# slowkoni/InStruct

Measured on AMD Instinct MI355X. Metric: MCMC iterations/sec (update_P+update_ZQ+update_SG) at NxLxK, higher is better.
Workload: dtype f64; 1 GPU; config3: N=10000 L=5000 K=5 diploid mode 2, 1 chain per GPU; N=10000, L=5000, K=5, ploidy=2, mode=2, rng_schedule=replay, chains=1, parallelism=1 independent chain(s), one per GPU

## Files before the change

### instruct_amd/csrc/isg_hip.hip

```cpp
#include <hip/hip_runtime.h>
#include <limits.h>
#include <math.h>
#include <stdint.h>
#include <stdio.h>
#include <stdlib.h>
#include <string.h>
#include <atomic>
#include <chrono>
#include <string>
#include <thread>
#include <vector>
#include <new>
#include <type_traits>
#include "../../include/instruct_hip.h"
#include "isg_math.h"
#include "isg_wh.h"
#include "isg_sampler.h"
#include "isg_host_dirichlet.h"
#include "isg_kdispatch.h"
#include "isg_devbuf.h"

#define ISG_KCAP 32
#define ISG_KWIDE 64
#define ISG_LPT 4

static thread_local std::string g_err;
static int fail(const std::string &m)
{
	g_err = m;
	return 1;
}
static bool env_flag(const char *e, bool def) { return e ? (def ? atoi(e) != 0 : atoi(e) == 1) : def; }
static long env_int(const char *e, long def, long lo = LONG_MIN, long hi = LONG_MAX) { return (e && atol(e) >= lo && atol(e) <= hi) ? atol(e) : def; }
static double env_double(const char *e, double def, double lo, double hi = HUGE_VAL) { return (e && atof(e) >= lo && atof(e) <= hi) ? atof(e) : def; }
#define HIPCHK(x)                                                                                     \
	do {                                                                                          \
		hipError_t e_ = (x);                                                                  \
		if (e_ != hipSuccess)                                                                 \
			return fail(std::string(#x) + ": " + hipGetErrorString(e_));                  \
	} while (0)

struct DevView {
	int N, L, Lp, K, KP, Amax, mode, type_freq;
	const uint8_t *geno;
	uint8_t *z;
	const int *allelenum;
	const int *nvalid;
	const unsigned *rankwave;
	int nwv;
	double *freq;
	float *freqf;
	int KPF;
	double *lftab, *lltab;
	int2 *lli;
	unsigned lli_F;
	const double *tape;
	unsigned long long tape_len;
	int *cnt;
	double *qq;
	int *qqnum;
	int *gen;
	int *genprop;
	double *uacc;
	double *indvlkh;
	const isg_wh_tables *tab;
	unsigned *err;
};

struct ProfEntry {
	std::string name;
	double ms;
	long n;
};
struct ProfPending {
	const char *name;
	hipEvent_t e0, e1;
};

struct PolyCtx;
struct InbreedCtx;
struct ResolveCtx;
struct PDevCtx;
struct SpecCtx;
template <class T>
struct PageAlloc {
	typedef T value_type;
	PageAlloc() {}
	template <class U> PageAlloc(const PageAlloc<U> &) {}
	T *allocate(size_t n)
	{
		void *p = nullptr;
		const size_t bytes = (n * sizeof(T) + 4095) & ~(size_t)4095;
		if (posix_memalign(&p, 4096, bytes ? bytes : 4096)) throw std::bad_alloc();
		return (T *)p;
	}
	void deallocate(T *p, size_t) { free(p); }
	template <class U> bool operator==(const PageAlloc<U> &) const { return true; }
	template <class U> bool operator!=(const PageAlloc<U> &) const { return false; }
};
template <class T> using hvec = std::vector<T, PageAlloc<T>>;

struct CoopBuf;
struct CtxBufs {
	DevBuf<uint8_t> d_geno, d_z;
	DevBuf<int> d_allelenum, d_nvalid, d_cnt, d_qqnum, d_gen, d_genprop;
	DevBuf<unsigned> d_rankwave;
	DevBuf<double> d_freq, d_lftab, d_lltab, d_qq, d_uacc, d_indvlkh;
	DevBuf<float> d_freqf;
	DevBuf<int2> d_lli;
	DevBuf<isg_wh_tables> d_tab;
	DevBuf<uint64_t> d_pos;
	DevBuf<unsigned> d_err;
	DevBuf<double> d_S;
	DevBuf<double> d_Fprop;
	DevBuf<double> d_tape;
	DevBuf<CoopBuf> d_coop;
	DevBuf<unsigned long long> d_pipe;
	DevBuf<unsigned long long> d_spop;
	DevBuf<double> d_qqsave;
	DevBuf<int> d_state;
	DevBuf<double> d_ratios, d_total;
	PinnedBuf<double> htape;
	DevEvent ev_tape;
	DevEvent ev_cnt;
	DevBuf<double> st_qq, st_qq2, st_lkh, st_gen, st_gen2, st_freq, st_freq2;
};
struct isg_ctx : CtxBufs {
	isg_config cfg;
	ResolveCtx *rs = nullptr;
	SpecCtx *zspec = nullptr;
	PDevCtx *pdev = nullptr;
	PolyCtx *poly = nullptr;
	InbreedCtx *inb = nullptr;
	DevView d;
	int Amax;
	hipStream_t stream;
	std::vector<int> allelenum;
	hvec<double> freq;
	hvec<double> qq;
	hvec<int> qqnum;
	hvec<int> gen;
	hvec<double> S;
	hvec<int> state;
	hvec<double> indvlkh;
	hvec<int> cnt_h;
	hvec<double> freq_stage;
	double alpha, totallkh;
	isg_wh rng;
	isg_wh origin;
	long raw_seed[3];
	bool raw_valid;
	uint64_t iter;
	uint64_t ky[9];
	isg_wh_tables tab_h;
	uint64_t nvalid_total;
	int coop;
	int spec;
	int xcd;
	int pipe;
	int pipe_xcd;
	bool counted = false;
	double host_t[8] = {0, 0, 0, 0, 0, 0, 0, 0};
	long host_n = 0;
	bool host_timing = false;
	std::vector<void *> pinned;
	bool ahead_valid = false;
	isg_wh ahead_rng;
	std::vector<double> pshape;
	std::vector<HostGammaCoef> pcoef;
	uint64_t htape_len = 0;
	int host_tape = 1;
	int spop_tree = 1;
	int test_abort = 0;
	long zq_fallbacks = 0;
	hvec<double> ratios_h;
	bool h_qq, h_gen, h_S, h_lkh;
	long st_step = 0;
	bool st_on = false;
	bool prof;
	std::vector<ProfEntry> prof_entries;
	std::vector<ProfPending> prof_pending;
	std::vector<hipEvent_t> prof_free;
	hipEvent_t prof_cur;
};


__device__ __forceinline__ unsigned lane_id() { return threadIdx.x & 63u; }

__device__ __forceinline__ unsigned wave_sum_u32(unsigned x)
{
	x += (unsigned)__builtin_amdgcn_update_dpp(0, (int)x, 0x121, 0xf, 0xf, false);
	x += (unsigned)__builtin_amdgcn_update_dpp(0, (int)x, 0x122, 0xf, 0xf, false);
	x += (unsigned)__builtin_amdgcn_update_dpp(0, (int)x, 0x124, 0xf, 0xf, false);
	x += (unsigned)__builtin_amdgcn_update_dpp(0, (int)x, 0x128, 0xf, 0xf, false);
	return (unsigned)__builtin_amdgcn_readlane((int)x, 0) + (unsigned)__builtin_amdgcn_readlane((int)x, 16) +
	       (unsigned)__builtin_amdgcn_readlane((int)x, 32) + (unsigned)__builtin_amdgcn_readlane((int)x, 48);
}


template <int BLOCK>
__device__ __forceinline__ unsigned block_excl_scan(unsigned v, unsigned *sm , unsigned *total)
{
	const int NW = BLOCK / 64;
	unsigned lane = lane_id(), w = threadIdx.x >> 6, incl = v;
#pragma unroll
	for (int o = 1; o < 64; o <<= 1) {
		unsigned t = __shfl_up(incl, o, 64);
		if (lane >= (unsigned)o) incl += t;
	}
	if (lane == 63) sm[w] = incl;
	__syncthreads();
	unsigned base = 0, tot = 0;
#pragma unroll
	for (int i = 0; i < NW; i++) {
		unsigned s = sm[i];
		if (i < (int)w) base += s;
		tot += s;
	}
	__syncthreads();
	*total = tot;
	return base + incl - v;
}

struct AccLimbs {
	unsigned long long l0, l1, l2, l3;
	unsigned flags;
};
__device__ __forceinline__ AccLimbs acc_to_limbs(const isg_acc &a)
{
	AccLimbs r;
	r.l0 = a.lo & 0xffffffffULL;
	r.l1 = a.lo >> 32;
	r.l2 = a.hi & 0xffffffffULL;
	r.l3 = a.hi >> 32;
	r.flags = a.flags;
	return r;
}
__device__ __forceinline__ isg_acc limbs_to_acc(const AccLimbs &s)
{
	isg_acc a;
	unsigned long long t0 = s.l0, t1 = s.l1 + (t0 >> 32), t2 = s.l2 + (t1 >> 32), t3 = s.l3 + (t2 >> 32);
	a.lo = (t0 & 0xffffffffULL) | (t1 << 32);
	a.hi = (t2 & 0xffffffffULL) | (t3 << 32);
	a.flags = s.flags;
	return a;
}
template <int BLOCK>
__device__ __forceinline__ isg_acc block_reduce_acc(const isg_acc &a, unsigned long long *sm )
{
	const int NW = BLOCK / 64;
	AccLimbs s = acc_to_limbs(a);
#pragma unroll
	for (int o = 32; o > 0; o >>= 1) {
		s.l0 += __shfl_down(s.l0, o, 64);
		s.l1 += __shfl_down(s.l1, o, 64);
		s.l2 += __shfl_down(s.l2, o, 64);
		s.l3 += __shfl_down(s.l3, o, 64);
		s.flags |= __shfl_down(s.flags, o, 64);
	}
	unsigned w = threadIdx.x >> 6;
	if (lane_id() == 0) {
		sm[w * 5 + 0] = s.l0;
		sm[w * 5 + 1] = s.l1;
		sm[w * 5 + 2] = s.l2;
		sm[w * 5 + 3] = s.l3;
		sm[w * 5 + 4] = s.flags;
	}
	__syncthreads();
	AccLimbs t = {0, 0, 0, 0, 0};
	for (int i = 0; i < NW; i++) {
		t.l0 += sm[i * 5 + 0];
		t.l1 += sm[i * 5 + 1];
		t.l2 += sm[i * 5 + 2];
		t.l3 += sm[i * 5 + 3];
		t.flags |= (unsigned)sm[i * 5 + 4];
	}
	__syncthreads();
	return limbs_to_acc(t);
}

template <int BLOCK, int LPT>
__global__ void __launch_bounds__(BLOCK) k_count(DevView d, int rows_per_block)
{
	extern __shared__ unsigned lds_cnt[];
	const int C = LPT * d.Amax * d.K;
	const int t = threadIdx.x;
	for (int c = 0; c < C; c++) lds_cnt[c * BLOCK + t] = 0;
	const int J0 = blockIdx.x * BLOCK * LPT;
	const int j0 = J0 + t * LPT;
	const int r0 = blockIdx.y * rows_per_block;
	int r1 = r0 + rows_per_block;
	if (r1 > d.N) r1 = d.N;
	const size_t rowb = (size_t)d.Lp * 2;
	if (j0 < d.Lp) {
		for (int i = r0; i < r1; i++) {
			unsigned long long gb, zb;
			if (LPT == 4) {
				const uint2 g = *(const uint2 *)(d.geno + (size_t)i * rowb + (size_t)j0 * 2);
				const uint2 zz = *(const uint2 *)(d.z + (size_t)i * rowb + (size_t)j0 * 2);
				gb = ((unsigned long long)g.y << 32) | g.x;
				zb = ((unsigned long long)zz.y << 32) | zz.x;
			} else {
				gb = *(const unsigned short *)(d.geno + (size_t)i * rowb + (size_t)j0 * 2);
				zb = *(const unsigned short *)(d.z + (size_t)i * rowb + (size_t)j0 * 2);
			}
#pragma unroll
			for (int l = 0; l < LPT; l++) {
				unsigned a0 = (unsigned)(gb >> (16 * l)) & 0xff, a1 = (unsigned)(gb >> (16 * l + 8)) & 0xff;
				unsigned z0 = (unsigned)(zb >> (16 * l)) & 0xff, z1 = (unsigned)(zb >> (16 * l + 8)) & 0xff;
				if (a0 != 0xff) {
					lds_cnt[((l * d.Amax + a0) * d.K + z0) * BLOCK + t] += 1;
					lds_cnt[((l * d.Amax + a1) * d.K + z1) * BLOCK + t] += 1;
				}
			}
		}
	}
	__syncthreads();
	const int per_locus = d.Amax * d.K;
	int tile_loci = d.L - J0;
	if (tile_loci > BLOCK * LPT) tile_loci = BLOCK * LPT;
	if (tile_loci < 0) tile_loci = 0;
	const int E = tile_loci * per_locus;
	for (int e = t; e < E; e += BLOCK) {
		int jl = e / per_locus, rem = e - jl * per_locus;
		unsigned v = lds_cnt[((jl % LPT) * per_locus + rem) * BLOCK + jl / LPT];
		if (v) atomicAdd(&d.cnt[(size_t)J0 * per_locus + e], (int)v);
	}
}

__global__ void k_count_atomic(DevView d)
{
	const size_t id = (size_t)blockIdx.x * blockDim.x + threadIdx.x;
	if (id >= (size_t)d.N * d.Lp) return;
	const unsigned short g = ((const unsigned short *)d.geno)[id], z = ((const unsigned short *)d.z)[id];
	const unsigned a0 = g & 0xff, a1 = g >> 8;
	if (a0 == 0xff) return;
	const size_t j = id % d.Lp;
	atomicAdd(&d.cnt[(j * d.Amax + a0) * d.K + (z & 0xff)], 1);
	atomicAdd(&d.cnt[(j * d.Amax + a1) * d.K + (z >> 8)], 1);
}

template <int BLOCK, int KC>
__device__ __forceinline__ void gprop_body(DevView d, const double *S, isg_wh base, int keyed, uint64_t *pos_out)
{
	__shared__ unsigned sm[BLOCK / 64 + 1];
	__shared__ double Ssh[KC];
	const bool indiv = (d.mode == 3);
	if (!indiv && threadIdx.x < (unsigned)d.K) Ssh[threadIdx.x] = S[threadIdx.x];
	__syncthreads();
	unsigned running = 0;
	for (int i0 = 0; i0 < d.N; i0 += BLOCK) {
		int i = i0 + threadIdx.x;
		double selfing = 0;
		int stat = 0;
		if (i < d.N) {
			if (indiv) selfing = S[i];
			else for (int k = 0; k < d.K; k++) selfing += d.qq[(size_t)i * d.K + k] * Ssh[k];
			stat = isg_dt_stat(selfing);
			if (stat < 0) {
				if ((atomicOr(d.err, 2u) & 2u) == 0u) *(double *)(d.err + 2) = selfing;
				stat = 1;
			}
		}
		unsigned flag = (i < d.N && stat == 1) ? 1u : 0u, tot, pre;
		pre = block_excl_scan<BLOCK>(flag, sm, &tot);
		if (i < d.N) {
			uint64_t pos = keyed ? 2ull * (uint64_t)i : (uint64_t)i + running + pre;
			isg_cursor c;
			c.s = isg_wh_jump(d.tab, base, pos);
			c.used = 0;
			c.tape = nullptr;
			int gen;
			if (stat == 1) {
				gen = isg_rgeom(&c, 1 - selfing);
				if (gen < 1) gen = 1;
				if (gen > 50) gen = 50;
			} else if (stat == 0) gen = 1;
			else gen = 50;
			d.genprop[i] = gen;
			d.uacc[i] = isg_cur_next(&c);
		}
		running += tot;
	}
	if (threadIdx.x == 0) *pos_out = (uint64_t)d.N + running;
}
template <int BLOCK>
__global__ void __launch_bounds__(BLOCK) k_gprop(DevView d, const double *S, isg_wh base, int keyed, uint64_t *pos_out) { gprop_body<BLOCK, ISG_KCAP>(d, S, base, keyed, pos_out); }
template <int BLOCK>
__global__ void __launch_bounds__(BLOCK) k_gprop_w(DevView d, const double *S, isg_wh base, int keyed, uint64_t *pos_out) { gprop_body<BLOCK, ISG_KWIDE>(d, S, base, keyed, pos_out); }

template <int BLOCK>
__device__ __forceinline__ isg_acc2 block_reduce_acc2(const isg_acc2 &a, long long *sm )
{
	const int NW = BLOCK / 64;
	long long hi = a.hi, lo = a.lo;
	unsigned fl = a.flags;
#pragma unroll
	for (int o = 32; o > 0; o >>= 1) {
		hi += __shfl_down(hi, o, 64);
		lo += __shfl_down(lo, o, 64);
		fl |= __shfl_down(fl, o, 64);
	}
	const unsigned w = threadIdx.x >> 6;
	if (lane_id() == 0) {
		sm[w * 3 + 0] = hi;
		sm[w * 3 + 1] = lo;
		sm[w * 3 + 2] = (long long)fl;
	}
	__syncthreads();
	isg_acc2 r;
	r.hi = 0;
	r.lo = 0;
	r.flags = 0;
	for (int i = 0; i < NW; i++) {
		r.hi += sm[i * 3 + 0];
		r.lo += sm[i * 3 + 1];
		r.flags |= (unsigned)sm[i * 3 + 2];
	}
	__syncthreads();
	return r;
}

__global__ void k_lltab(DevView d)
{
	const size_t id = (size_t)blockIdx.x * blockDim.x + threadIdx.x;
	const size_t per = (size_t)d.L * d.Amax * d.Amax * d.K;
	if (id >= per) return;
	const int k = (int)(id % d.K);
	const int a1 = (int)((id / d.K) % d.Amax), a0 = (int)((id / d.K / d.Amax) % d.Amax), j = (int)(id / d.K / d.Amax / d.Amax);
	const double f0 = d.freq[((size_t)j * d.Amax + a0) * d.KP + k], f1 = d.freq[((size_t)j * d.Amax + a1) * d.KP + k];
	if (a1 == 0) d.lftab[((size_t)j * d.Amax + a0) * d.K + k] = isg_log(f0);
	if (!d.lltab || d.mode != 2) return;
	if (a0 == a1) {
		double result = f0 * f0, temp = 2 * f0 * (1 - f0);
		for (int g = 1; g <= 50; g++) {
			d.lltab[(size_t)(g - 1) * per + id] = isg_log(result);
			temp /= 2;
			result += temp / 2;
		}
	} else {
		for (int g = 1; g <= 50; g++) d.lltab[(size_t)(g - 1) * per + id] = isg_log(2 * f0 * f1 * isg_scalbn(1.0, -(g - 1)));
	}
}

__device__ __forceinline__ int2 lli_entry(double v)
{
	if (!(v > -1024.0 && v < 1024.0)) {
		const uint64_t u = isg_d2u(v);
		return make_int2((int)0x80000000u, (u == 0x7ff0000000000000ULL) ? 1 : (u == 0xfff0000000000000ULL) ? 2 : 4);
	}
	const double hs = __builtin_rint(v * 1048576.0);
	const double lo = isg_fma(hs, -0x1p-20, v);
	return make_int2((int)hs, (int)__builtin_rint(lo * 0x1p51));
}
__global__ void k_lltab_int(DevView d)
{
	const size_t id = (size_t)blockIdx.x * blockDim.x + threadIdx.x;
	const size_t AAK = (size_t)d.Amax * d.Amax * d.K;
	if (id == 0) d.lli[0] = make_int2(0, 0);
	if (id >= AAK * d.L) return;
	const int j = (int)(id % d.L), combo = (int)(id / d.L);
	const int k = combo % d.K, a1 = (combo / d.K) % d.Amax, a0 = combo / d.K / d.Amax;
	const double f0 = d.freq[((size_t)j * d.Amax + a0) * d.KP + k], f1 = d.freq[((size_t)j * d.Amax + a1) * d.KP + k];
	if (a1 == 0) d.lli[d.lli_F + ((size_t)a0 * d.K + k) * d.Lp + j] = lli_entry(isg_log(f0));
	int2 *out = d.lli + 1 + (size_t)combo * d.Lp + j;
	const size_t gstride = AAK * d.Lp;
	if (a0 == a1) {
		double result = f0 * f0, temp = 2 * f0 * (1 - f0);
		for (int g = 1; g <= 50; g++) {
			out[(size_t)(g - 1) * gstride] = lli_entry(isg_log(result));
			temp /= 2;
			result += temp / 2;
		}
	} else {
		for (int g = 1; g <= 50; g++) out[(size_t)(g - 1) * gstride] = lli_entry(isg_log(2 * f0 * f1 * isg_scalbn(1.0, -(g - 1))));
	}
}

// ... 960 lines not shown
	if (a == 2) return (b == 2 || b == 1) ? 0.5 : 0.0;
	if (a == 1) return (b == 0 || b == 2) ? 0.05 : (b == 1 ? 0.90 : 0.0);
	return 0.0;
}
template <int BLOCK>
__device__ __forceinline__ double dev_proposal(const DevView &d, const double *s, unsigned long long *smr)
{
	isg_acc a;
	isg_acc_zero(&a);
	for (int i = threadIdx.x; i < d.N; i += BLOCK) {
		double temp = 0;
		for (int j = 0; j < d.K; j++) temp += d.qq[(size_t)i * d.K + j] * s[j];
		isg_acc_add(&a, isg_log(isg_pow(temp, (double)(d.gen[i] - 1)) * (1 - temp)));
	}
	const isg_acc r = block_reduce_acc<BLOCK>(a, smr);
	return isg_acc_value(&r);
}
template <int BLOCK, int KC>
__device__ __forceinline__ void spop_body(DevView d, double *S, int *state, isg_wh start, int back_refl, uint64_t *used_out)
{
	__shared__ unsigned long long smr[(BLOCK / 64) * 5];
	__shared__ double Scur[KC], Stmp[KC];
	__shared__ int stc[KC], stt[KC];
	__shared__ double ld_sh;
	const int t = threadIdx.x, K = d.K;
	if (t < K) { Scur[t] = S[t]; stc[t] = state[t]; }
	__syncthreads();
	double cur_ld = dev_proposal<BLOCK>(d, Scur, smr);
	isg_cursor c;
	c.s = start;
	c.used = 0;
	c.tape = nullptr;
	for (int j = 0; j < K; j++) {
		if (t == 0) {
			for (int i = 0; i < K; i++) { Stmp[i] = Scur[i]; stt[i] = stc[i]; }
			if (back_refl == 1) {
				double v = isg_cur_next(&c) * 2 * 0.05 - 0.05;
				v += Scur[j];
				if (v <= 0.0) v = 0.0 - v;
				else if (v >= 1.0) v = 1.0 - (v - 1.0);
				Stmp[j] = v;
			} else {
				const int st = stc[j];
				double v;
				int ns;
				if (st == 0) {
					if (isg_cur_next(&c) < 0.50) { v = 0.0; ns = 0; } else { v = isg_cur_next(&c); ns = 1; }
				} else if (st == 2) {
					if (isg_cur_next(&c) < 0.5) { v = 1.0; ns = 2; } else { v = isg_cur_next(&c); ns = 1; }
				} else {
					const double tt = isg_cur_next(&c);
					if (tt <= 0.05) { v = 0.0; ns = 0; }
					else if (tt >= 0.95) { v = 1.0; ns = 2; }
					else { v = isg_cur_next(&c); ns = 1; }
				}
				Stmp[j] = v;
				stt[j] = ns;
			}
		}
		__syncthreads();
		const double new_ld = dev_proposal<BLOCK>(d, Stmp, smr);
		if (t == 0) {
			double mh = isg_exp(new_ld - cur_ld);
			if (back_refl == 0) {
				double h = 1.0;
				for (int i = 0; i < K; i++) h *= dev_q_trans(stc[i], stt[i]) / dev_q_trans(stt[i], stc[i]);
				mh *= h;
			}
			const double thr = (1 > mh) ? mh : 1;
			double keep = cur_ld;
			if (isg_cur_next(&c) < thr) {
				Scur[j] = Stmp[j];
				if (back_refl == 0) stc[j] = stt[j];
				keep = new_ld;
			}
			ld_sh = keep;
		}
		__syncthreads();
		cur_ld = ld_sh;
	}
	if (t < K) { S[t] = Scur[t]; state[t] = stc[t]; }
	if (t == 0) *used_out = c.used;
}
template <int BLOCK>
__global__ void __launch_bounds__(BLOCK) k_spop(DevView d, double *S, int *state, isg_wh start, int back_refl, uint64_t *used_out) { spop_body<BLOCK, ISG_KCAP>(d, S, state, start, back_refl, used_out); }
template <int BLOCK>
__global__ void __launch_bounds__(BLOCK) k_spop_w(DevView d, double *S, int *state, isg_wh start, int back_refl, uint64_t *used_out) { spop_body<BLOCK, ISG_KWIDE>(d, S, state, start, back_refl, used_out); }

#define ISG_SPOP_TREE_K 6
__device__ __forceinline__ double spop_proposed(double cur, double u)
{
	double v = u * 2 * 0.05 - 0.05;
	v += cur;
	if (v <= 0.0) v = 0.0 - v;
	else if (v >= 1.0) v = 1.0 - (v - 1.0);
	return v;
}
__global__ void __launch_bounds__(256) k_spop_tree(DevView d, const double *S, isg_wh start, unsigned long long *limbs )
{
	__shared__ double Scur[ISG_SPOP_TREE_K], V[ISG_SPOP_TREE_K];
	const int K = d.K, t = threadIdx.x;
	if (t < K) {
		Scur[t] = S[t];
		isg_wh s = isg_wh_jump(d.tab, start, 2ull * (unsigned)t);
		V[t] = spop_proposed(Scur[t], isg_wh_next(&s));
	}
	__syncthreads();
	const int i = blockIdx.x * 256 + t;
	double q[ISG_SPOP_TREE_K];
	double gm1 = 0.0;
#pragma unroll
	for (int m = 0; m < ISG_SPOP_TREE_K; m++) q[m] = (i < d.N && m < K) ? d.qq[(size_t)i * K + m] : 0.0;
	if (i < d.N) gm1 = (double)(d.gen[i] - 1);
	{
		const int e = blockIdx.y;
		int j = -1, h = 0;
		if (e) {
			j = 31 - __builtin_clz((unsigned)e);
			h = e - (1 << j);
		}
		isg_acc a;
		isg_acc_zero(&a);
		if (i < d.N) {
			double temp = 0;
#pragma unroll
			for (int m = 0; m < ISG_SPOP_TREE_K; m++)
				if (m < K) temp += q[m] * ((m == j || (m < j && ((h >> m) & 1))) ? V[m] : Scur[m]);
			isg_acc_add(&a, isg_log(isg_pow(temp, gm1) * (1 - temp)));
		}
		AccLimbs sl = acc_to_limbs(a);
#pragma unroll
		for (int o = 32; o > 0; o >>= 1) {
			sl.l0 += __shfl_down(sl.l0, o, 64);
			sl.l1 += __shfl_down(sl.l1, o, 64);
			sl.l2 += __shfl_down(sl.l2, o, 64);
			sl.l3 += __shfl_down(sl.l3, o, 64);
			sl.flags |= __shfl_down(sl.flags, o, 64);
		}
		if (lane_id() == 0) {
			atomicAdd(&limbs[e * 5 + 0], sl.l0);
			atomicAdd(&limbs[e * 5 + 1], sl.l1);
			atomicAdd(&limbs[e * 5 + 2], sl.l2);
			atomicAdd(&limbs[e * 5 + 3], sl.l3);
			if (sl.flags) atomicOr(&limbs[e * 5 + 4], (unsigned long long)sl.flags);
		}
	}
}
__global__ void k_spop_decide(DevView d, double *S, isg_wh start, const unsigned long long *limbs)
{
	if (threadIdx.x || blockIdx.x) return;
	const int K = d.K;
	auto value = [&](int e) {
		AccLimbs sl;
		sl.l0 = limbs[e * 5 + 0];
		sl.l1 = limbs[e * 5 + 1];
		sl.l2 = limbs[e * 5 + 2];
		sl.l3 = limbs[e * 5 + 3];
		sl.flags = (unsigned)limbs[e * 5 + 4];
		const isg_acc a = limbs_to_acc(sl);
		return isg_acc_value(&a);
	};
	double cur_ld = value(0);
	int h = 0;
	isg_cursor c;
	c.s = isg_wh_jump(d.tab, start, 0);
	c.used = 0;
	c.tape = nullptr;
	for (int j = 0; j < K; j++) {
		const double v = spop_proposed(S[j], isg_cur_next(&c));
		const double new_ld = value((1 << j) + h);
		const double mh = isg_exp(new_ld - cur_ld);
		const double thr = (1 > mh) ? mh : 1;
		if (isg_cur_next(&c) < thr) {
			S[j] = v;
			h |= 1 << j;
			cur_ld = new_ld;
		}
	}
}

__global__ void k_alpha_ratios(DevView d, double ralpha, double alpha, double *ratios)
{
	const size_t id = (size_t)blockIdx.x * blockDim.x + threadIdx.x;
	if (id >= (size_t)d.N * d.K) return;
	const double q = d.qq[id], n = (double)d.qqnum[id];
	ratios[id] = isg_pow(q, ralpha + n) / isg_pow(q, n + alpha);
}

template <int BLOCK>
__global__ void __launch_bounds__(BLOCK) k_lkh_total(DevView d, double *total)
{
	__shared__ unsigned long long smr[(BLOCK / 64) * 5];
	isg_acc a;
	isg_acc_zero(&a);
	for (int i = threadIdx.x; i < d.N; i += BLOCK) isg_acc_add(&a, d.indvlkh[i]);
	const isg_acc r = block_reduce_acc<BLOCK>(a, smr);
	if (threadIdx.x == 0) *total = isg_acc_value(&r);
}


static void prof_collect(isg_ctx *c)
{
	for (auto &p : c->prof_pending) {
		(void)hipEventSynchronize(p.e1);
		float ms = 0;
		(void)hipEventElapsedTime(&ms, p.e0, p.e1);
		bool found = false;
		for (auto &e : c->prof_entries)
			if (e.name == p.name) {
				e.ms += ms;
				e.n++;
				found = true;
				break;
			}
		if (!found) c->prof_entries.push_back({p.name, (double)ms, 1});
		c->prof_free.push_back(p.e0);
		c->prof_free.push_back(p.e1);
	}
	c->prof_pending.clear();
}
static hipEvent_t prof_event(isg_ctx *c)
{
	if (c->prof_free.empty()) {
		if (c->prof_pending.size() >= 2048) prof_collect(c);
		if (c->prof_free.empty()) {
			hipEvent_t e;
			(void)hipEventCreate(&e);
			return e;
		}
	}
	hipEvent_t e = c->prof_free.back();
	c->prof_free.pop_back();
	return e;
}
static void prof_begin(isg_ctx *c)
{
	if (!c->prof) return;
	c->prof_cur = prof_event(c);
	(void)hipEventRecord(c->prof_cur, c->stream);
}
static void prof_end(isg_ctx *c, const char *name)
{
	if (!c->prof) return;
	hipEvent_t e1 = prof_event(c);
	(void)hipEventRecord(e1, c->stream);
	c->prof_pending.push_back({name, c->prof_cur, e1});
}

static int report_dev_err(const unsigned e[4])
{
	if (e[0] & 2u) {
		double v;
		char msg[160];
		memcpy(&v, e + 2, sizeof(v));
		snprintf(msg, sizeof(msg), "The value of selfing rate or inbreeding coefficient %f is beyond [0,1]!", v);
		return fail(msg);
	}
	if (e[0]) return fail("device error flag set");
	return 0;
}

static int refresh_freqf(isg_ctx *c);
static void keyed_layout(isg_ctx *c)
{
	uint64_t N = c->cfg.N, L = c->cfg.L, P = c->cfg.P, K = c->cfg.K, A = c->Amax;
	uint64_t SP = 16 * A + 16, SZ = P * L + 16 * K + 16, ZI0 = 1 + 2 * N, B0 = ZI0 + N * SZ;
	uint64_t offS = K * L * SP, offG = offS + 4 * K, offZ = offG + 2 * N, offA = offZ + N * SZ, BLK = offA + 4;
	if (c->cfg.mode == 3) BLK += 2 * N;
	uint64_t v[9] = {SP, SZ, ZI0, B0, offS, offG, offZ, offA, BLK};
	memcpy(c->ky, v, sizeof(v));
}
enum { KY_SP, KY_SZ, KY_ZI0, KY_B0, KY_OFFS, KY_OFFG, KY_OFFZ, KY_OFFA, KY_BLK };
static bool is_keyed(const isg_ctx *c) { return c->cfg.rng_sched == ISG_SCHED_KEYED; }
static uint64_t iter_base(const isg_ctx *c) { return c->ky[KY_B0] + c->iter * c->ky[KY_BLK]; }

static double host_next(isg_ctx *c)
{
	c->raw_valid = false;
	return isg_wh_next(&c->rng);
}
static void host_seek(isg_ctx *c, uint64_t pos) { c->rng = isg_wh_jump(&c->tab_h, c->origin, pos); c->raw_valid = false; }
static void host_advance(isg_ctx *c, uint64_t n) { c->rng = isg_wh_jump(&c->tab_h, c->rng, n); c->raw_valid = false; }

static int host_tape_begin(isg_ctx *c, uint64_t ngamma)
{
	c->htape_len = 0;
	const uint64_t need = host_tape_need(ngamma, c->host_tape != 0);
	if (!need) return 0;
	HIPCHK(c->d_tape.grow(need));
	HIPCHK(c->htape.grow(need));
	prof_begin(c);
	hipLaunchKernelGGL(k_tape, dim3((unsigned)((need + 2047) / 2048)), dim3(256), 0, c->stream, c->d.tab, c->rng, (unsigned long long)need, c->d_tape);
	prof_end(c, "k_tape_host");
	HIPCHK(hipGetLastError());
	HIPCHK(hipMemcpyAsync(c->htape, c->d_tape, sizeof(double) * need, hipMemcpyDeviceToHost, c->stream));
	c->htape_len = need;
	return 0;
}
static void pin_host(isg_ctx *c, void *ptr, size_t bytes)
{
	if (ptr && bytes && hipHostRegister(ptr, bytes, hipHostRegisterDefault) == hipSuccess) c->pinned.push_back(ptr);
	else (void)hipGetLastError();
}
#define HOST_T(c, k, t0) do { if ((c)->host_timing) { const auto t1_ = std::chrono::steady_clock::now(); (c)->host_t[k] += std::chrono::duration<double>(t1_ - (t0)).count(); (t0) = t1_; } } while (0)
enum { HOSTP_REQUEST = 1, HOSTP_DRAW = 2 };
struct HostPSecond { const int *d_cnt; int *cnt_h; double *freq_h; };
static int host_update_P(isg_ctx *c, int halves, const int *d_cnt, const HostPSecond *second, bool skip_single)
{
	auto ht0 = std::chrono::steady_clock::now();
	const HostDirichletPass pass = {c->allelenum.data(), c->cfg.K, c->cfg.L, c->Amax, skip_single, second ? 2 : 1,
					{c->cnt_h.data(), second ? second->cnt_h : nullptr}, {c->freq.data(), second ? second->freq_h : nullptr}};
	const uint64_t ngamma = ngamma_of(pass);
	if (halves & HOSTP_REQUEST) {
		HIPCHK(hipMemcpyAsync(c->cnt_h.data(), d_cnt, sizeof(int) * c->cnt_h.size(), hipMemcpyDeviceToHost, c->stream));
		if (second) HIPCHK(hipMemcpyAsync(second->cnt_h, second->d_cnt, sizeof(int) * c->cnt_h.size(), hipMemcpyDeviceToHost, c->stream));
		if (!c->ev_cnt) HIPCHK(hipEventCreateWithFlags(&c->ev_cnt.e, hipEventDisableTiming));
		HIPCHK(hipEventRecord(c->ev_cnt, c->stream));
		if (host_tape_begin(c, ngamma)) return 1;
		if (!(halves & HOSTP_DRAW)) {
			if (!c->ev_tape) HIPCHK(hipEventCreateWithFlags(&c->ev_tape.e, hipEventDisableTiming));
			HIPCHK(hipEventRecord(c->ev_tape, c->stream));
			c->ahead_rng = c->rng;
			c->ahead_valid = true;
			return 0;
		}
	}
	HIPCHK(hipEventSynchronize(c->ev_cnt));
	HOST_T(c, 0, ht0);
	c->pshape.resize(ngamma);
	c->pcoef.resize(ngamma);
	host_pass_shapes(pass, c->pshape.data());
	HOST_T(c, 1, ht0);
	host_gamma_coefs(c->pshape.data(), (size_t)ngamma, c->pcoef.data());
	HOST_T(c, 2, ht0);
	if (halves & HOSTP_REQUEST) HIPCHK(hipStreamSynchronize(c->stream));
	else HIPCHK(hipEventSynchronize(c->ev_tape));
	HOST_T(c, 3, ht0);
	const HostTape tape = {c->htape, c->htape_len, c->rng, &c->tab_h};
	c->rng = host_pass_draw(pass, c->pshape.data(), c->pcoef.data(), tape);
	c->raw_valid = false;
	HOST_T(c, 4, ht0);
	return 0;
}

extern "C" const char *isg_last_error(void) { return g_err.c_str(); }
extern "C" long isg_diag_live_buffers(void) { return g_live_buffers.load(); }

template <class Kern>
static bool fits_resident(Kern kern, int threads, long blocks, int device)
{
	int per_cu = 0, cus = 0;
	if (hipOccupancyMaxActiveBlocksPerMultiprocessor(&per_cu, kern, threads, 0) != hipSuccess) return false;
	if (hipDeviceGetAttribute(&cus, hipDeviceAttributeMultiprocessorCount, device) != hipSuccess) return false;
	return (long)per_cu * cus >= blocks;
}
static std::atomic<int> g_live_ctx[64];
static void ctx_count(isg_ctx *c, int delta);
#include "isg_resolve_hip.inc"
#include "isg_walk_hip.inc"
#include "isg_spec_hip.inc"
static void ctx_count(isg_ctx *c, int delta)
{
	if (c->cfg.device < 0) return;
	if (delta > 0 && !c->counted) { g_live_ctx[c->cfg.device & 63].fetch_add(1); c->counted = true; }
	if (delta < 0 && c->counted) { g_live_ctx[c->cfg.device & 63].fetch_sub(1); c->counted = false; }
}

static int poly_ctx_create(const isg_config *cfg, const int32_t *allelenum, const int32_t *seq, isg_ctx **out);
static int poly_update_P(isg_ctx *c);
static int poly_update_S_POP(isg_ctx *c);
static int poly_update_ZQ(isg_ctx *c, int init_flag);
static int poly_cal_lkh(isg_ctx *c);
static int poly_count_alleles(isg_ctx *c, int32_t *counts);
extern "C" void isg_ctx_destroy(isg_ctx *c);
static int noadm_update_Z(isg_ctx *c, int init_flag);
static int noadm_cal_lkh(isg_ctx *c);
static int indiv_update_S_IND(isg_ctx *c);
static int indiv_update_F_IND(isg_ctx *c);
static int indiv_cal_lkh_F(isg_ctx *c);
static int inbreed_update_F_POP(isg_ctx *c);
static int inbreed_cal_lkh(isg_ctx *c);
static int inbreed_alloc(isg_ctx *c);
#define NOT_POLY(c, what) if ((c)->poly) return fail(what ": not part of the ploidy 4 chain (poly_geno.c:98-116)")

static int ctx_init_common(isg_ctx *c, const std::vector<int> &nvalid, int Lp, int KP, size_t nS)
{
	const int N = c->cfg.N, L = c->cfg.L, K = c->cfg.K, Amax = c->Amax;
	c->freq.assign((size_t)K * L * Amax, 0.0);
	c->freq_stage.assign((size_t)Lp * Amax * KP, 0.0);
	c->qq.assign((size_t)N * K, 0.0);
	c->qqnum.assign((size_t)N * K, 0);
	c->gen.assign(N, 0);
	c->S.assign(nS, 0.0);
	c->state.assign(K, 0);
	c->indvlkh.assign(N, 0.0);
	c->cnt_h.assign((size_t)L * Amax * K, 0);
	pin_host(c, c->cnt_h.data(), sizeof(int) * c->cnt_h.size());
	pin_host(c, c->freq_stage.data(), sizeof(double) * c->freq_stage.size());
	c->nvalid_total = 0;
	for (int i = 0; i < N; i++) c->nvalid_total += (uint64_t)nvalid[i];
	c->alpha = 0;
	c->totallkh = 0;
	c->iter = 0;
	c->rng.s1 = 13; c->rng.s2 = 4; c->rng.s3 = 1972;
	c->origin = c->rng;
	c->raw_seed[0] = 13; c->raw_seed[1] = 4; c->raw_seed[2] = 1972;
	c->raw_valid = true;
	c->prof = false;
	c->host_timing = env_flag(getenv("INSTRUCT_HOST_TIMING"), false);
	c->host_tape = env_flag(getenv("INSTRUCT_HOST_TAPE"), true);
	c->h_qq = c->h_gen = c->h_S = c->h_lkh = true;
	isg_wh_tables_init(&c->tab_h);
	HIPCHK(c->d_tab.upload(&c->tab_h, 1));
	HIPCHK(c->d_pos.alloc_zero(4));
	HIPCHK(c->d_err.alloc_zero(4));
	c->d.tab = c->d_tab;
	c->d.err = c->d_err;
	return 0;
}

struct CtxGuard {
	isg_ctx *c;
	explicit CtxGuard(isg_ctx *p) : c(p) {}
	~CtxGuard() { if (c) isg_ctx_destroy(c); }
	void release() { c = nullptr; }
};
extern "C" int isg_ctx_create(const isg_config *cfg, const int32_t *allelenum, const int32_t *geno, const int32_t *missindx, isg_ctx **out)
{
	*out = nullptr;
	if (cfg->P == 4) return fail("isg_ctx_create: ploidy 4 data goes through isg_ctx_create_poly");
	if (cfg->P != 2) return fail("isg_ctx_create: only ploidy 2 and 4 are supported");
	if (cfg->K < 1 || cfg->K > ISG_KWIDE) return fail("isg_ctx_create: K must be in 1..64 for ploidy 2");
	if (cfg->mode < 0 || cfg->mode > 5) return fail("isg_ctx_create: mode must be 0 .. 5");
	if (cfg->N < 1 || cfg->L < 1) return fail("isg_ctx_create: empty problem");
	int ndev = 0;
	if (hipGetDeviceCount(&ndev) != hipSuccess || ndev == 0) return fail("isg_ctx_create: no HIP device available (the MI355X path has no CPU fallback)");
	if (cfg->device < 0 || cfg->device >= ndev) return fail("isg_ctx_create: bad device ordinal");
	HIPCHK(hipSetDevice(cfg->device));
	isg_ctx *c = new isg_ctx();
	c->cfg = *cfg;
	ctx_count(c, +1);
	memset(&c->d, 0, sizeof(c->d));
	CtxGuard guard(c);
	const int N = cfg->N, L = cfg->L, K = cfg->K;
	int Amax = 0;
	for (int j = 0; j < L; j++) Amax = allelenum[j] > Amax ? allelenum[j] : Amax;
	if (Amax > 254) return fail("isg_ctx_create: more than 254 alleles at a locus");
	if (Amax < 1) Amax = 1;
	c->Amax = Amax;
	const int Lp = (L + 7) & ~7, KP = (K + 1) & ~1;
	c->allelenum.assign(allelenum, allelenum + L);
	std::vector<uint8_t> pk((size_t)N * Lp * 2, 0xff);
	std::vector<int> nvalid(N, 0);
	for (int i = 0; i < N; i++)
		for (int j = 0; j < L; j++) {
			if (missindx[(size_t)i * L + j] == 1 || allelenum[j] <= 1) continue;
			int a0 = geno[((size_t)i * L + j) * 2], a1 = geno[((size_t)i * L + j) * 2 + 1];
			if (a0 < 0 || a1 < 0 || a0 >= allelenum[j] || a1 >= allelenum[j]) return fail("isg_ctx_create: allele code out of range at a non-missing locus");
			pk[((size_t)i * Lp + j) * 2] = (uint8_t)a0;
			pk[((size_t)i * Lp + j) * 2 + 1] = (uint8_t)a1;
			nvalid[i]++;
		}
	DevView &d = c->d;
	memset(&d, 0, sizeof(d));
	d.N = N; d.L = L; d.Lp = Lp; d.K = K; d.KP = KP; d.Amax = Amax; d.mode = cfg->mode; d.type_freq = cfg->type_freq;
	HIPCHK(hipStreamCreate(&c->stream));
	HIPCHK(c->d_geno.upload(pk));
	d.geno = c->d_geno;
	HIPCHK(c->d_z.alloc_zero((size_t)N * Lp * 2));
	d.z = c->d_z;
	HIPCHK(hipMemset(d.z, 0xff, (size_t)N * Lp * 2));
	HIPCHK(c->d_allelenum.upload(allelenum, L));
	d.allelenum = c->d_allelenum;
	HIPCHK(c->d_nvalid.upload(nvalid));
	d.nvalid = c->d_nvalid;
	HIPCHK(c->d_freq.alloc_zero((size_t)Lp * Amax * KP));
	d.freq = c->d_freq;
	d.KPF = (K + 3) & ~3;
	HIPCHK(c->d_freqf.alloc_zero((size_t)Lp * Amax * d.KPF));
	d.freqf = c->d_freqf;
	if (cfg->type_freq == 1 || cfg->mode == 0) {
		if (env_flag(getenv("INSTRUCT_LL_TABLES"), true)) {
			HIPCHK(c->d_lftab.alloc_zero((size_t)L * Amax * K));
			const size_t ent = (size_t)50 * L * Amax * Amax * K;
			const size_t enti = 1 + (size_t)50 * Lp * Amax * Amax * K + (size_t)Lp * Amax * K;
			if (cfg->mode == 2 && env_flag(getenv("INSTRUCT_LL_INT"), true) && enti * sizeof(int2) <= ((size_t)1 << 30)) {
				HIPCHK(c->d_lli.alloc_zero(enti));
				d.lli_F = (unsigned)(1 + (size_t)50 * Lp * Amax * Amax * K);
			} else if (cfg->mode == 2 && ent * sizeof(double) <= ((size_t)1 << 30)) { HIPCHK(c->d_lltab.alloc_zero(ent)); }
			if (cfg->mode == 4) {
				size_t fr = 0, tot = 0;
				if (hipMemGetInfo(&fr, &tot) != hipSuccess) fr = (size_t)1 << 31;
				if ((ent / 50) * sizeof(double) <= fr / 2) { HIPCHK(c->d_lltab.alloc_zero(ent / 50)); }
			}
			d.lftab = c->d_lftab; d.lltab = c->d_lltab; d.lli = c->d_lli;
		}
	}
	if (resolve_alloc(c, nvalid)) return 1;
	if (cfg->rng_sched == ISG_SCHED_REPLAY && pdev_create(c, &c->pdev, L, K, Amax, allelenum, 1)) return 1;
	if (cfg->rng_sched == ISG_SCHED_REPLAY && cfg->mode != 0 && spec_create(c, &c->zspec, nvalid, 2)) return 1;
	{
		const int nwv = (Lp + 63) / 64 + 1;
		std::vector<unsigned> rw((size_t)N * nwv, 0);
		for (int i = 0; i < N; i++) {
			unsigned run = 0;
			for (int w = 0; w < nwv; w++) {
				rw[(size_t)i * nwv + w] = run;
				for (int j = 64 * w; j < 64 * (w + 1) && j < Lp; j++) run += (pk[((size_t)i * Lp + j) * 2] != 0xff) ? 1u : 0u;
			}
		}
		HIPCHK(c->d_rankwave.upload(rw));
		d.rankwave = c->d_rankwave;
		d.nwv = nwv;
	}
	{
		HIPCHK(c->d_coop.alloc_zero(1));
		c->coop = env_flag(getenv("INSTRUCT_ZQ_COOP"), true);
		c->spec = env_flag(getenv("INSTRUCT_ZQ_SPEC"), true);
		c->xcd = env_flag(getenv("INSTRUCT_ZQ_XCD"), false);
		c->pipe = env_flag(getenv("INSTRUCT_ZQ_PIPE"), true);
		c->spop_tree = env_flag(getenv("INSTRUCT_SPOP_TREE"), true);
		c->pipe_xcd = env_flag(getenv("INSTRUCT_ZQ_PIPE_XCD"), true);
		c->test_abort = (int)env_int(getenv("INSTRUCT_ZQ_TEST_ABORT"), 0);
	}
	HIPCHK(c->d_cnt.alloc_zero((size_t)Lp * Amax * K));
	HIPCHK(c->d_qq.alloc_zero((size_t)N * K));
	HIPCHK(c->d_qqsave.alloc_zero((size_t)N * K));
	HIPCHK(c->d_qqnum.alloc_zero((size_t)N * K));
	HIPCHK(c->d_gen.alloc_zero(N));
	HIPCHK(c->d_genprop.alloc_zero(N));
	HIPCHK(c->d_uacc.alloc_zero(N));
	HIPCHK(c->d_indvlkh.alloc_zero(N));
	d.cnt = c->d_cnt; d.qq = c->d_qq; d.qqnum = c->d_qqnum; d.gen = c->d_gen; d.genprop = c->d_genprop; d.uacc = c->d_uacc; d.indvlkh = c->d_indvlkh;
	const bool per_indiv = cfg->mode == 3 || cfg->mode == 5;
	if (ctx_init_common(c, nvalid, Lp, KP, per_indiv ? N : K)) return 1;
	HIPCHK(c->d_S.alloc_zero(per_indiv && N > ISG_KWIDE ? N : ISG_KWIDE));
	if (cfg->mode == 5) HIPCHK(c->d_Fprop.alloc_zero(N));
	HIPCHK(c->d_state.alloc_zero(ISG_KWIDE));
	HIPCHK(c->d_ratios.alloc_zero((size_t)N * K));
	HIPCHK(c->d_total.alloc_zero(1));
	c->ratios_h.assign((size_t)N * K, 0.0);
	keyed_layout(c);
	if (cfg->mode == 0 && !d.lftab) return fail("isg_ctx_create: mode 0 needs its log frequency table (INSTRUCT_LL_TABLES must not be 0)");
	if (cfg->mode == 4) {
		if (!d.lltab) return fail("isg_ctx_create: mode 4 needs its log-likelihood table (INSTRUCT_LL_TABLES must not be 0; L * Amax^2 * K doubles, at most half of the free device memory)");
		if (inbreed_alloc(c)) return 1;
	}
	guard.release();
	*out = c;
	return 0;
}

extern "C" int isg_set_seeds(isg_ctx *c, long s1, long s2, long s3)
{
	if (s1 < 0 || s2 < 0 || s3 < 0) return fail("isg_set_seeds: negative seeds are not supported");
	c->rng.s1 = (uint32_t)(s1 % ISG_M1); c->rng.s2 = (uint32_t)(s2 % ISG_M2); c->rng.s3 = (uint32_t)(s3 % ISG_M3);
	c->raw_seed[0] = s1; c->raw_seed[1] = s2; c->raw_seed[2] = s3;
	c->raw_valid = true;
	return 0;
}
extern "C" int isg_get_seeds(isg_ctx *c, long s[3])
{
	if (c->raw_valid) { s[0] = c->raw_seed[0]; s[1] = c->raw_seed[1]; s[2] = c->raw_seed[2]; }
	else { s[0] = c->rng.s1; s[1] = c->rng.s2; s[2] = c->rng.s3; }
	return 0;
}
extern "C" double isg_ran1(isg_ctx *c) { return host_next(c); }

extern "C" int isg_keyed_layout(isg_ctx *c, uint64_t out[9])
{
	memcpy(out, c->ky, sizeof(c->ky));
	return 0;
}

static int upload_freq(isg_ctx *c)
{
	const int L = c->cfg.L, K = c->cfg.K, A = c->Amax, KP = c->d.KP;
	freq_to_device(c->freq.data(), c->freq_stage.data(), K, L, A, KP);
	HIPCHK(hipMemcpyAsync(c->d.freq, c->freq_stage.data(), sizeof(double) * (size_t)L * A * KP, hipMemcpyHostToDevice, c->stream));
	return refresh_freqf(c);
}
static int refresh_freqf(isg_ctx *c)
{
	DevView &d = c->d;
	size_t n = (size_t)d.L * d.Amax * d.KPF;
	prof_begin(c);
	hipLaunchKernelGGL(k_freqf, dim3((unsigned)((n + 255) / 256)), dim3(256), 0, c->stream, d);
	prof_end(c, "k_freqf");
	if (d.lli) {
		const size_t per = (size_t)d.L * d.Amax * d.Amax * d.K;
		prof_begin(c);
		hipLaunchKernelGGL(k_lltab_int, dim3((unsigned)((per + 127) / 128)), dim3(128), 0, c->stream, d);
		prof_end(c, "k_lltab");
	} else if (d.lftab) {
		const size_t per = (size_t)d.L * d.Amax * d.Amax * d.K;
		prof_begin(c);
		hipLaunchKernelGGL(k_lltab, dim3((unsigned)((per + 127) / 128)), dim3(128), 0, c->stream, d);
		prof_end(c, "k_lltab");
	}
	HIPCHK(hipGetLastError());
	return 0;
}
static int download_freq(isg_ctx *c)
{
	const int L = c->cfg.L, K = c->cfg.K, A = c->Amax, KP = c->d.KP;
	HIPCHK(hipMemcpyAsync(c->freq_stage.data(), c->d.freq, sizeof(double) * (size_t)L * A * KP, hipMemcpyDeviceToHost, c->stream));
	HIPCHK(hipStreamSynchronize(c->stream));
	freq_from_device(c->freq_stage.data(), c->freq.data(), K, L, A, KP);
	return 0;
}
static int ensure_qq(isg_ctx *c)
{
	if (c->h_qq) return 0;
	HIPCHK(hipMemcpyAsync(c->qq.data(), c->d.qq, sizeof(double) * c->qq.size(), hipMemcpyDeviceToHost, c->stream));
	HIPCHK(hipMemcpyAsync(c->qqnum.data(), c->d.qqnum, sizeof(int) * c->qqnum.size(), hipMemcpyDeviceToHost, c->stream));
	HIPCHK(hipStreamSynchronize(c->stream));
	c->h_qq = true;
	return 0;
}
static int ensure_gen(isg_ctx *c)
{
	if (c->h_gen) return 0;
	HIPCHK(hipMemcpyAsync(c->gen.data(), c->d.gen, sizeof(int) * c->gen.size(), hipMemcpyDeviceToHost, c->stream));
	HIPCHK(hipStreamSynchronize(c->stream));
	c->h_gen = true;
	return 0;
}
static int ensure_S(isg_ctx *c)
{
	if (c->h_S) return 0;
	HIPCHK(hipMemcpyAsync(c->S.data(), c->d_S, sizeof(double) * c->S.size(), hipMemcpyDeviceToHost, c->stream));
	HIPCHK(hipMemcpyAsync(c->state.data(), c->d_state, sizeof(int) * c->cfg.K, hipMemcpyDeviceToHost, c->stream));
	HIPCHK(hipStreamSynchronize(c->stream));
	c->h_S = true;
	return 0;
}
static int ensure_lkh(isg_ctx *c)
{
	if (c->h_lkh) return 0;
	unsigned e[4] = {0, 0, 0, 0};
	HIPCHK(hipMemcpyAsync(c->indvlkh.data(), c->d.indvlkh, sizeof(double) * c->indvlkh.size(), hipMemcpyDeviceToHost, c->stream));
	HIPCHK(hipMemcpyAsync(&c->totallkh, c->d_total, sizeof(double), hipMemcpyDeviceToHost, c->stream));
	if (!c->poly) HIPCHK(hipMemcpyAsync(e, c->d_err, sizeof(e), hipMemcpyDeviceToHost, c->stream));
	HIPCHK(hipStreamSynchronize(c->stream));
	if (report_dev_err(e)) return 1;
	c->h_lkh = true;
	return 0;
}

template <int BLOCK, int LPT>
static int launch_count_tile(isg_ctx *c)
{
	DevView &d = c->d;
	const size_t lds = (size_t)LPT * d.Amax * d.K * BLOCK * sizeof(unsigned);
	int tiles = (d.Lp + BLOCK * LPT - 1) / (BLOCK * LPT);
	int rb = (1024 + tiles - 1) / tiles;
	if (rb > d.N) rb = d.N;
	if (rb < 1) rb = 1;
	int rows = (d.N + rb - 1) / rb;
	rb = (d.N + rows - 1) / rows;
	HIPCHK(hipFuncSetAttribute((const void *)k_count<BLOCK, LPT>, hipFuncAttributeMaxDynamicSharedMemorySize, 160 * 1024));
	prof_begin(c);
	hipLaunchKernelGGL((k_count<BLOCK, LPT>), dim3(tiles, rb), dim3(BLOCK), lds, c->stream, d, rows);
	prof_end(c, "k_count");
	return 0;
}
static int launch_count(isg_ctx *c)
{
	DevView &d = c->d;
	HIPCHK(hipMemsetAsync(d.cnt, 0, sizeof(int) * (size_t)d.L * d.Amax * d.K, c->stream));
	const size_t per_lane = (size_t)d.Amax * d.K * sizeof(unsigned);
	const size_t cap = 150 * 1024;
	if (4 * per_lane * 256 <= cap) { if (launch_count_tile<256, 4>(c)) return 1; }
	else if (per_lane * 256 <= cap) { if (launch_count_tile<256, 1>(c)) return 1; }
	else if (per_lane * 64 <= cap) { if (launch_count_tile<64, 1>(c)) return 1; }
	else {
		const size_t n = (size_t)d.N * d.Lp;
		prof_begin(c);
		hipLaunchKernelGGL(k_count_atomic, dim3((unsigned)((n + 255) / 256)), dim3(256), 0, c->stream, d);
		prof_end(c, "k_count_atomic");
	}
	HIPCHK(hipGetLastError());
	return 0;
}

extern "C" int isg_count_alleles(isg_ctx *c, int32_t *counts)
{
	HIPCHK(hipSetDevice(c->cfg.device));
	if (c->poly) return poly_count_alleles(c, counts);
	if (launch_count(c)) return 1;
	HIPCHK(hipMemcpyAsync(c->cnt_h.data(), c->d.cnt, sizeof(int) * c->cnt_h.size(), hipMemcpyDeviceToHost, c->stream));
	HIPCHK(hipStreamSynchronize(c->stream));
	counts_from_device(c->cnt_h.data(), nullptr, counts, c->cfg.K, c->cfg.L, c->Amax);
	return 0;
}

static int update_P_ahead(isg_ctx *c)
{
	c->ahead_valid = false;
	if (c->poly || is_keyed(c) || !c->host_tape) return 0;
	if (c->pdev && c->pdev->usable) return 0;
	if (launch_count(c)) return 1;
	return host_update_P(c, HOSTP_REQUEST, c->d.cnt, nullptr, true);
}

extern "C" int isg_update_P(isg_ctx *c)
{
	HIPCHK(hipSetDevice(c->cfg.device));
	if (c->poly) return poly_update_P(c);
	DevView &d = c->d;
	const int L = c->cfg.L, K = c->cfg.K;
	const bool ahead = c->ahead_valid && !is_keyed(c) && c->ahead_rng.s1 == c->rng.s1 && c->ahead_rng.s2 == c->rng.s2 && c->ahead_rng.s3 == c->rng.s3;
	c->ahead_valid = false;
	if (!ahead && launch_count(c)) return 1;
	if (is_keyed(c)) {
		int n = K * L, B = 256;
		prof_begin(c);
		hipLaunchKernelGGL(k_pdirich, dim3((n + B - 1) / B), dim3(B), 0, c->stream, d, c->origin, iter_base(c), c->ky[KY_SP]);
		prof_end(c, "k_pdirich");
		HIPCHK(hipGetLastError());
		return refresh_freqf(c);
	}
	if (!ahead && c->pdev && c->pdev->usable) {
		bool done = false;
		if (pdev_update_P(c, c->pdev, &done)) return 1;
		if (done) return refresh_freqf(c);
	}
	if (host_update_P(c, ahead ? HOSTP_DRAW : HOSTP_REQUEST | HOSTP_DRAW, d.cnt, nullptr, true)) return 1;
	auto ht0 = std::chrono::steady_clock::now();
	const int rc_up = upload_freq(c);
	HOST_T(c, 5, ht0);
	c->host_n++;
	return rc_up;
}

extern "C" int isg_update_S_POP(isg_ctx *c)
{
	if (c->cfg.mode == 4 && !c->poly) {
		HIPCHK(hipSetDevice(c->cfg.device));
		return inbreed_update_F_POP(c);
	}
	if (c->cfg.mode != 2) return 0;
	HIPCHK(hipSetDevice(c->cfg.device));
	if (c->poly) return poly_update_S_POP(c);
	const int K = c->cfg.K;
	isg_wh start = is_keyed(c) ? isg_wh_jump(&c->tab_h, c->origin, iter_base(c) + c->ky[KY_OFFS]) : c->rng;
	if (c->cfg.back_refl == 1 && K <= ISG_SPOP_TREE_K && c->spop_tree) {
		const size_t nb = sizeof(unsigned long long) * 5 * ((size_t)1 << K);
		if (!c->d_spop) HIPCHK(c->d_spop.alloc(5 * ((size_t)1 << ISG_SPOP_TREE_K)));
		HIPCHK(hipMemsetAsync(c->d_spop, 0, nb, c->stream));
		prof_begin(c);
		hipLaunchKernelGGL(k_spop_tree, dim3((c->cfg.N + 255) / 256, 1u << K), dim3(256), 0, c->stream, c->d, (const double *)c->d_S, start, c->d_spop);
		hipLaunchKernelGGL(k_spop_decide, dim3(1), dim3(64), 0, c->stream, c->d, c->d_S, start, (const unsigned long long *)c->d_spop);
		prof_end(c, "k_spop");
	} else {
		prof_begin(c);
		if (K > ISG_KCAP) hipLaunchKernelGGL(k_spop_w<1024>, dim3(1), dim3(1024), 0, c->stream, c->d, c->d_S, c->d_state, start, c->cfg.back_refl, c->d_pos + 1);
		else hipLaunchKernelGGL(k_spop<1024>, dim3(1), dim3(1024), 0, c->stream, c->d, c->d_S, c->d_state, start, c->cfg.back_refl, c->d_pos + 1);
		prof_end(c, "k_spop");
	}
	HIPCHK(hipGetLastError());
	c->h_S = false;
	if (!is_keyed(c)) {
		uint64_t used = 2ull * (uint64_t)K;
		if (c->cfg.back_refl == 0) {
			HIPCHK(hipMemcpyAsync(&used, c->d_pos + 1, sizeof(used), hipMemcpyDeviceToHost, c->stream));
			HIPCHK(hipStreamSynchronize(c->stream));
		}
		host_advance(c, used);
	}
	return 0;
}

extern "C" int isg_update_G(isg_ctx *c)
{
	NOT_POLY(c, "isg_update_G");
	if (c->cfg.mode != 2 && c->cfg.mode != 3) return 0;
	HIPCHK(hipSetDevice(c->cfg.device));
	DevView &d = c->d;
	double *d_S = c->d_S;
	isg_wh base = is_keyed(c) ? isg_wh_jump(&c->tab_h, c->origin, iter_base(c) + c->ky[KY_OFFG]) : c->rng;
	prof_begin(c);
	if (d.K > ISG_KCAP) hipLaunchKernelGGL(k_gprop_w<1024>, dim3(1), dim3(1024), 0, c->stream, d, (const double *)d_S, base, is_keyed(c) ? 1 : 0, c->d_pos);
	else hipLaunchKernelGGL(k_gprop<1024>, dim3(1), dim3(1024), 0, c->stream, d, (const double *)d_S, base, is_keyed(c) ? 1 : 0, c->d_pos);
	prof_end(c, "k_gprop");
	prof_begin(c);
	if (d.lli && d.mode == 2) hipLaunchKernelGGL((k_loglik_int<256, true>), dim3(d.N), dim3(256), 0, c->stream, d);
	else if (d.lltab) hipLaunchKernelGGL((k_loglik_tab<256, true>), dim3(d.N), dim3(256), 0, c->stream, d);
	else if (d.K > ISG_KCAP) hipLaunchKernelGGL((k_loglik_w<256, true>), dim3(d.N), dim3(256), 0, c->stream, d);
	else hipLaunchKernelGGL((k_loglik<256, true>), dim3(d.N), dim3(256), 0, c->stream, d);
	prof_end(c, "k_loglik_pair");
	HIPCHK(hipGetLastError());
	c->h_gen = false;
	if (!is_keyed(c)) {
		uint64_t used = 0;
		unsigned e[4] = {0, 0, 0, 0};
		HIPCHK(hipMemcpyAsync(&used, c->d_pos, sizeof(used), hipMemcpyDeviceToHost, c->stream));
		HIPCHK(hipMemcpyAsync(e, c->d_err, sizeof(e), hipMemcpyDeviceToHost, c->stream));
		HIPCHK(hipStreamSynchronize(c->stream));
		if (report_dev_err(e)) return 1;
		host_advance(c, used);
	}
	return 0;
}

static bool coop_sweep_failed(isg_ctx *c, const unsigned flags[2])
{
	bool bad = flags[0] || flags[1];
	if (c->test_abort > 0 && --c->test_abort == 0) bad = true;
	return bad;
}
static int tape_fill(isg_ctx *c, isg_wh base, uint64_t need)
{
	HIPCHK(c->d_tape.grow(need));
	if (need) {
		prof_begin(c);
		hipLaunchKernelGGL(k_tape, dim3((unsigned)((need + 2047) / 2048)), dim3(256), 0, c->stream, c->d.tab, base, (unsigned long long)need, c->d_tape);
		prof_end(c, "k_tape");
	}
	c->d.tape = c->d_tape;
	c->d.tape_len = need;
	return 0;
}
static int coop_sweep_end(isg_ctx *c, bool launched, bool *done)
{
	uint64_t used = 0;
	unsigned flags[2] = {0, 0};
	HIPCHK(hipMemcpyAsync(&used, c->d_pos, sizeof(used), hipMemcpyDeviceToHost, c->stream));
	HIPCHK(hipMemcpyAsync(flags, &((CoopBuf *)c->d_coop)->abort_flag, sizeof(flags), hipMemcpyDeviceToHost, c->stream));
	HIPCHK(hipStreamSynchronize(c->stream));
	*done = launched && !coop_sweep_failed(c, flags);
	if (*done) {
		host_advance(c, used);
		c->h_qq = false;
		return 0;
	}
	HIPCHK(hipMemcpyAsync(c->d.qq, c->d_qqsave, sizeof(double) * (size_t)c->cfg.N * c->cfg.K, hipMemcpyDeviceToDevice, c->stream));
	c->zq_fallbacks++;
	return 0;
}
static int chain_sweep_end(isg_ctx *c)
{
	uint64_t used = 0;
	HIPCHK(hipMemcpyAsync(&used, c->d_pos, sizeof(used), hipMemcpyDeviceToHost, c->stream));
	HIPCHK(hipStreamSynchronize(c->stream));
	host_advance(c, used);
	return 0;
}
template <int KMAX>
static void launch_zq(isg_ctx *c, bool chain, isg_wh base, uint64_t pos0, uint64_t stride, int init_flag)
{
	DevView &d = c->d;
	if (chain)
		hipLaunchKernelGGL((k_zq<512, KMAX, true>), dim3(1), dim3(512), 0, c->stream, d, base, pos0, stride, init_flag, c->alpha, c->d_pos);
	else
		hipLaunchKernelGGL((k_zq<256, KMAX, false>), dim3(d.N), dim3(256), 0, c->stream, d, base, pos0, stride, init_flag, c->alpha, c->d_pos);
}
extern "C" int isg_update_ZQ(isg_ctx *c, int init_flag)
{
	c->ahead_valid = false;
	HIPCHK(hipSetDevice(c->cfg.device));
	if (c->poly) return poly_update_ZQ(c, init_flag);
	const int K = c->cfg.K;
	bool chain = !is_keyed(c);
	isg_wh base = chain ? c->rng : c->origin;
	uint64_t pos0 = chain ? 0 : (init_flag ? c->ky[KY_ZI0] : iter_base(c) + c->ky[KY_OFFZ]);
	uint64_t stride = c->ky[KY_SZ];
	c->d.tape = nullptr;
	c->d.tape_len = 0;
	if (chain && !init_flag && c->zspec) {
		bool done = false;
		if (spec_update_ZQ(c, c->zspec, base, &done)) return 1;
		if (done) return 0;
	}
	if (chain && !init_flag && c->rs) {
		bool done = false;
		if (resolve_update_ZQ(c, base, &done)) return 1;
		if (done) return 0;
	}
	if (chain) {
		uint64_t need = 2 * c->nvalid_total + (uint64_t)(8 * K + 32 > 96 ? 8 * K + 32 : 96) * (uint64_t)c->cfg.N + 4096;
		if (tape_fill(c, base, need)) return 1;
		HIPCHK(hipGetLastError());
	}
	const bool coop = chain && c->coop && K <= ISG_KCAP;
	if (coop) {
		HIPCHK(hipMemsetAsync(c->d_coop, 0, sizeof(CoopBuf), c->stream));
		int G = (c->d.Lp + 255) / 256;
		if (G > ISG_COOP_GMAX) G = ISG_COOP_GMAX;
		CoopBuf *cb = (CoopBuf *)c->d_coop;
		const int pack = (G <= 32 && c->xcd) ? 1 : 0;
		const bool spec = !init_flag && K <= 8 && G * 256 >= c->d.Lp && c->spec;
		const int GP = (c->d.Lp + 64 * ISG_PIPE_DW - 1) / (64 * ISG_PIPE_DW);
		const bool pipe = spec && c->pipe && !pack && 2 * c->d.Lp < 65536 && GP * ISG_PIPE_DW <= 64 * ISG_PIPE_RMAX && GP <= 192;
		const int ppack = (GP <= 32 && c->pipe_xcd) ? 1 : 0;
		if (pipe) {
			const size_t need_words = (size_t)ISG_COOP_RING * GP * ISG_PIPE_DW * ISG_PIPE_STRIDE;
			HIPCHK(c->d_pipe.grow(need_words));
			HIPCHK(hipMemsetAsync(c->d_pipe, 0, need_words * sizeof(unsigned long long), c->stream));
		}
		HIPCHK(hipMemcpyAsync(c->d_qqsave, c->d.qq, sizeof(double) * (size_t)c->cfg.N * K, hipMemcpyDeviceToDevice, c->stream));
		bool launched = true;
		prof_begin(c);
		if (pipe)
			kdispatch(KL_ZQ_8(), K, [&](auto km) {
				constexpr int KM = decltype(km)::value;
				if (fits_resident(k_zq_pipe<KM, ISG_PIPE_DW>, 64 * (ISG_PIPE_DW + 1), GP, c->cfg.device))
					hipLaunchKernelGGL((k_zq_pipe<KM, ISG_PIPE_DW>), dim3(ppack ? 8 * GP : GP), dim3(64 * (ISG_PIPE_DW + 1)), 0, c->stream, c->d, base, c->alpha, cb, c->d_pipe, c->d_pos, ppack);
				else launched = false;
			});
		else if (spec)
			kdispatch(KL_ZQ_8(), K, [&](auto km) {
				constexpr int KM = decltype(km)::value;
				if (fits_resident(k_zq_spec<KM>, 256, G, c->cfg.device))
					hipLaunchKernelGGL((k_zq_spec<KM>), dim3(pack ? 8 * G : G), dim3(256), 0, c->stream, c->d, base, c->alpha, cb, c->d_pos, pack);
				else launched = false;
			});
		else
			kdispatch(KL_ZQ_COOP(), K, [&](auto km) {
				constexpr int KM = decltype(km)::value;
				if (fits_resident(k_zq_coop<KM>, 256, G, c->cfg.device))
					hipLaunchKernelGGL((k_zq_coop<KM>), dim3(pack ? 8 * G : G), dim3(256), 0, c->stream, c->d, base, init_flag, c->alpha, cb, c->d_pos, pack);
				else launched = false;
			});
		prof_end(c, pipe ? "k_zq_pipe" : spec ? "k_zq_spec" : "k_zq_coop");
		HIPCHK(hipGetLastError());
		bool done = false;
		if (coop_sweep_end(c, launched, &done)) return 1;
		if (done) return 0;
	}
	prof_begin(c);
	kdispatch(KL_ZQ(), K, [&](auto km) { launch_zq<decltype(km)::value>(c, chain, base, pos0, stride, init_flag); });
	prof_end(c, chain ? "k_zq_chain" : "k_zq_keyed");
	HIPCHK(hipGetLastError());
	if (chain && chain_sweep_end(c)) return 1;
	c->h_qq = false;
	return 0;
}

extern "C" int isg_update_alpha(isg_ctx *c)
{
	NOT_POLY(c, "isg_update_alpha");
	HIPCHK(hipSetDevice(c->cfg.device));
	const size_t NK = (size_t)c->cfg.N * c->cfg.K;
	if (is_keyed(c)) host_seek(c, iter_base(c) + c->ky[KY_OFFA]);
	isg_cursor cur;
	cur.s = c->rng;
	cur.used = 0;
	cur.tape = nullptr;
	double ralpha = isg_rnormal(&cur, c->alpha, 1.0);
	c->rng = cur.s;
	c->raw_valid = false;
	if (ralpha > 0) {
		prof_begin(c);
		hipLaunchKernelGGL(k_alpha_ratios, dim3((unsigned)((NK + 255) / 256)), dim3(256), 0, c->stream, c->d, ralpha, c->alpha, c->d_ratios);
		prof_end(c, "k_alpha_ratios");
		HIPCHK(hipGetLastError());
		HIPCHK(hipMemcpyAsync(c->ratios_h.data(), c->d_ratios, sizeof(double) * NK, hipMemcpyDeviceToHost, c->stream));
		HIPCHK(hipStreamSynchronize(c->stream));
		double mh = 1.0;
		for (size_t k = 0; k < NK; k++) mh *= c->ratios_h[k];
		double thr = (1 > mh) ? mh : 1;
		c->alpha = (host_next(c) < thr) ? ralpha : c->alpha;
	}
	return update_P_ahead(c);
}

extern "C" int isg_cal_lkh(isg_ctx *c)
{
	HIPCHK(hipSetDevice(c->cfg.device));
	if (c->poly) return poly_cal_lkh(c);
	if (c->cfg.mode == 0) return noadm_cal_lkh(c);
	if (c->cfg.mode == 4) return inbreed_cal_lkh(c);
	if (c->cfg.mode == 5) return indiv_cal_lkh_F(c);
	DevView &d = c->d;
	prof_begin(c);
	if (d.lli && d.mode == 2) hipLaunchKernelGGL((k_loglik_int<256, false>), dim3(d.N), dim3(256), 0, c->stream, d);
	else if (d.lltab || (d.lftab && d.mode == 1)) hipLaunchKernelGGL((k_loglik_tab<256, false>), dim3(d.N), dim3(256), 0, c->stream, d);
	else if (d.K > ISG_KCAP) hipLaunchKernelGGL((k_loglik_w<256, false>), dim3(d.N), dim3(256), 0, c->stream, d);
	else hipLaunchKernelGGL((k_loglik<256, false>), dim3(d.N), dim3(256), 0, c->stream, d);
	prof_end(c, "k_loglik_lkh");
	prof_begin(c);
	hipLaunchKernelGGL(k_lkh_total<1024>, dim3(1), dim3(1024), 0, c->stream, d, c->d_total);
	prof_end(c, "k_lkh_total");
	HIPCHK(hipGetLastError());
	c->h_lkh = false;
	return 0;
}

#include "isg_poly_hip.inc"
#include "isg_modes_hip.inc"

extern "C" void isg_ctx_destroy(isg_ctx *c)
{
	if (!c) return;
	ctx_count(c, -1);
	if (c->host_timing && c->host_n > 0)
		fprintf(stderr, "replay update_P host side, ms per sweep over %ld sweeps: counts %.3f  shapes %.3f  constants %.3f  tape %.3f  draws %.3f  upload %.3f\n", c->host_n,
			1e3 * c->host_t[0] / c->host_n, 1e3 * c->host_t[1] / c->host_n, 1e3 * c->host_t[2] / c->host_n, 1e3 * c->host_t[3] / c->host_n, 1e3 * c->host_t[4] / c->host_n, 1e3 * c->host_t[5] / c->host_n);
	(void)hipSetDevice(c->cfg.device);
	(void)hipStreamSynchronize(c->stream);
	for (void *q : c->pinned) (void)hipHostUnregister(q);
	c->pinned.clear();
	delete c->rs;
	delete c->pdev;
	delete c->zspec;
	delete c->poly;
	delete c->inb;
	static_cast<CtxBufs &>(*c) = CtxBufs();
	prof_collect(c);
	for (auto e : c->prof_free) (void)hipEventDestroy(e);
	(void)hipStreamDestroy(c->stream);
	delete c;
}

extern "C" int isg_update_Z(isg_ctx *c, int init_flag)
{
	c->ahead_valid = false;
	if (c->poly || c->cfg.mode != 0) return fail("isg_update_Z: mode 0 (-v 0) only");
	HIPCHK(hipSetDevice(c->cfg.device));
	return noadm_update_Z(c, init_flag);
}

extern "C" int isg_update_S_IND(isg_ctx *c)
{
	if (c->poly || (c->cfg.mode != 3 && c->cfg.mode != 5)) return fail("isg_update_S_IND: modes 3 and 5 (-v 3, -v 5) only");
	HIPCHK(hipSetDevice(c->cfg.device));
	return c->cfg.mode == 3 ? indiv_update_S_IND(c) : indiv_update_F_IND(c);
}

extern "C" int isg_iteration(isg_ctx *c)
{
	if (is_keyed(c) && iter_base(c) + c->ky[KY_BLK] >= (1ull << 52)) return fail("isg_iteration: the keyed schedule's stream positions reach 2^52 (the generator's period is 6.95e12 anyway)");
	if (c->poly) {
		HIPCHK(hipSetDevice(c->cfg.device));
		return poly_iteration(c);
	}
	if (isg_update_P(c)) return 1;
	if (c->cfg.mode == 0) {
		if (isg_update_Z(c, 0)) return 1;
		if (isg_cal_lkh(c)) return 1;
		c->iter++;
		return 0;
	}
	if (c->cfg.mode == 2) {
		if (isg_update_S_POP(c)) return 1;
		if (isg_update_G(c)) return 1;
	}
	if (c->cfg.mode == 4 && isg_update_S_POP(c)) return 1;
	if (c->cfg.mode == 3) {
		if (isg_update_S_IND(c)) return 1;
		if (isg_update_G(c)) return 1;
	}
	if (c->cfg.mode == 5 && isg_update_S_IND(c)) return 1;
	if (isg_update_ZQ(c, 0)) return 1;
	if (isg_update_alpha(c)) return 1;
	if (isg_cal_lkh(c)) return 1;
	c->iter++;
	return 0;
}
extern "C" int isg_iter_advance(isg_ctx *c) { c->iter++; return 0; }
extern "C" int isg_run(isg_ctx *c, long n)
{
	for (long i = 0; i < n; i++)
		if (isg_iteration(c)) return 1;
	return 0;
}

extern "C" int isg_chain_init(isg_ctx *c, const float *initd)
{
	c->ahead_valid = false;
	HIPCHK(hipSetDevice(c->cfg.device));
	if (c->poly) return poly_chain_init(c, initd);
	const int N = c->cfg.N, K = c->cfg.K;
	c->origin = c->rng;
	c->iter = 0;
	HIPCHK(hipMemsetAsync(c->d_err, 0, 4 * sizeof(unsigned), c->stream));
	if (c->cfg.mode == 0) return isg_update_Z(c, 1);
	c->alpha = host_next(c) * 10;
	if (c->cfg.mode == 2) {
		isg_cursor cur;
		cur.s = c->rng;
		cur.used = 0;
	cur.tape = nullptr;
		for (int i = 0; i < N; i++) {
			double pr = isg_cur_next(&cur);
			int g = isg_rgeom(&cur, pr);
			if (g > 50) g = 50;
			c->gen[i] = g;
		}
		c->rng = cur.s;
		for (int k = 0; k < K; k++) {
			c->S[k] = (double)initd[k];
			if (c->cfg.back_refl == 0) {
				int st = isg_dt_stat(c->S[k]);
				if (st < 0) return fail("The value of selfing rate or inbreeding coefficient is beyond [0,1]!");
				c->state[k] = st;
			}
		}
		HIPCHK(hipMemcpyAsync(c->d.gen, c->gen.data(), sizeof(int) * N, hipMemcpyHostToDevice, c->stream));
		HIPCHK(hipMemcpyAsync(c->d_S, c->S.data(), sizeof(double) * K, hipMemcpyHostToDevice, c->stream));
		HIPCHK(hipMemcpyAsync(c->d_state, c->state.data(), sizeof(int) * K, hipMemcpyHostToDevice, c->stream));
		HIPCHK(hipStreamSynchronize(c->stream));
		c->h_gen = c->h_S = true;
	}
	if (c->cfg.mode == 3) {
		if (is_keyed(c)) {
			for (int i = 0; i < N; i++) {
				host_seek(c, 1 + 2 * (uint64_t)i);
				c->S[i] = host_next(c);
				c->gen[i] = isg_rgeom_u(host_next(c), 1 - c->S[i]);
			}
		} else {
			for (int i = 0; i < N; i++) c->S[i] = host_next(c);
			for (int i = 0; i < N; i++) c->gen[i] = isg_rgeom_u(host_next(c), 1 - c->S[i]);
		}
		HIPCHK(hipMemcpyAsync(c->d.gen, c->gen.data(), sizeof(int) * N, hipMemcpyHostToDevice, c->stream));
		HIPCHK(hipMemcpyAsync(c->d_S, c->S.data(), sizeof(double) * N, hipMemcpyHostToDevice, c->stream));
		HIPCHK(hipStreamSynchronize(c->stream));
		c->h_gen = c->h_S = true;
	}
	if (c->cfg.mode == 5) {
		for (int i = 0; i < N; i++) {
			if (is_keyed(c)) host_seek(c, 1 + 2 * (uint64_t)i);
			c->S[i] = host_next(c);
		}
		HIPCHK(hipMemcpyAsync(c->d_S, c->S.data(), sizeof(double) * N, hipMemcpyHostToDevice, c->stream));
		HIPCHK(hipStreamSynchronize(c->stream));
		c->h_S = true;
	}
	if (c->cfg.mode == 4) {
		for (int k = 0; k < K; k++) {
			c->S[k] = (double)initd[k];
			if (c->cfg.back_refl == 0) {
				int st = isg_dt_stat(c->S[k]);
				if (st < 0) return fail("The value of selfing rate or inbreeding coefficient is beyond [0,1]!");
				c->state[k] = st;
			}
		}
		HIPCHK(hipMemcpyAsync(c->d_S, c->S.data(), sizeof(double) * K, hipMemcpyHostToDevice, c->stream));
		HIPCHK(hipMemcpyAsync(c->d_state, c->state.data(), sizeof(int) * K, hipMemcpyHostToDevice, c->stream));
		HIPCHK(hipStreamSynchronize(c->stream));
		c->h_S = true;
	}
	return isg_update_ZQ(c, 1);
}

extern "C" int isg_get_amax(isg_ctx *c, int32_t *a) { *a = c->Amax; return 0; }
extern "C" int isg_get_z(isg_ctx *c, int32_t *z)
{
	HIPCHK(hipSetDevice(c->cfg.device));
	if (c->poly) return poly_get_bytes(c, c->poly->p.z, z);
	const int N = c->cfg.N, L = c->cfg.L, Lp = c->d.Lp;
	std::vector<uint8_t> h((size_t)N * Lp * 2);
	HIPCHK(hipMemcpyAsync(h.data(), c->d.z, h.size(), hipMemcpyDeviceToHost, c->stream));
	HIPCHK(hipStreamSynchronize(c->stream));
	bytes_to_ints(h.data(), z, N, L, Lp, 2);
	return 0;
}
extern "C" int isg_set_z(isg_ctx *c, const int32_t *z)
{
	c->ahead_valid = false;
	NOT_POLY(c, "isg_set_z");
	HIPCHK(hipSetDevice(c->cfg.device));
	const int N = c->cfg.N, L = c->cfg.L, Lp = c->d.Lp;
	std::vector<uint8_t> h((size_t)N * Lp * 2, 0xff);
	for (int i = 0; i < N; i++)
		for (int j = 0; j < L; j++)
			for (int k = 0; k < 2; k++) {
				int v = z[((size_t)i * L + j) * 2 + k];
				h[((size_t)i * Lp + j) * 2 + k] = (v < 0) ? 0xff : (uint8_t)v;
			}
	HIPCHK(hipMemcpy(c->d.z, h.data(), h.size(), hipMemcpyHostToDevice));
	return 0;
}
extern "C" int isg_get_freq(isg_ctx *c, double *f)
{
	HIPCHK(hipSetDevice(c->cfg.device));
	if (c->poly && c->poly->freq_host) { memcpy(f, c->freq.data(), sizeof(double) * c->freq.size()); return 0; }
	if (download_freq(c)) return 1;
	memcpy(f, c->freq.data(), sizeof(double) * c->freq.size());
	return 0;
}
extern "C" int isg_set_freq(isg_ctx *c, const double *f)
{
	NOT_POLY(c, "isg_set_freq");
	HIPCHK(hipSetDevice(c->cfg.device));
	memcpy(c->freq.data(), f, sizeof(double) * c->freq.size());
	if (upload_freq(c)) return 1;
	HIPCHK(hipStreamSynchronize(c->stream));
	return 0;
}
extern "C" int isg_get_qq(isg_ctx *c, double *q)
{
	HIPCHK(hipSetDevice(c->cfg.device));
	if (ensure_qq(c)) return 1;
	memcpy(q, c->qq.data(), sizeof(double) * c->qq.size());
	return 0;
}
extern "C" int isg_set_qq(isg_ctx *c, const double *q)
{
	HIPCHK(hipSetDevice(c->cfg.device));
	if (ensure_qq(c)) return 1;
	memcpy(c->qq.data(), q, sizeof(double) * c->qq.size());
	HIPCHK(hipMemcpy(c->d.qq, q, sizeof(double) * c->qq.size(), hipMemcpyHostToDevice));
	return 0;
}
extern "C" int isg_get_qqnum(isg_ctx *c, double *q)
{
	HIPCHK(hipSetDevice(c->cfg.device));
	if (ensure_qq(c)) return 1;
	for (size_t i = 0; i < c->qqnum.size(); i++) q[i] = (double)c->qqnum[i];
	return 0;
}
extern "C" int isg_get_generation(isg_ctx *c, int32_t *g)
{
	NOT_POLY(c, "isg_get_generation");
	HIPCHK(hipSetDevice(c->cfg.device));
	if (ensure_gen(c)) return 1;
	memcpy(g, c->gen.data(), sizeof(int) * c->gen.size());
	return 0;
}
extern "C" int isg_set_generation(isg_ctx *c, const int32_t *g)
{
	NOT_POLY(c, "isg_set_generation");
	HIPCHK(hipSetDevice(c->cfg.device));
	memcpy(c->gen.data(), g, sizeof(int) * c->gen.size());
	HIPCHK(hipMemcpy(c->d.gen, g, sizeof(int) * c->gen.size(), hipMemcpyHostToDevice));
	c->h_gen = true;
	return 0;
}
extern "C" int isg_get_self_rates(isg_ctx *c, double *s)
{
	HIPCHK(hipSetDevice(c->cfg.device));
	if (ensure_S(c)) return 1;
	memcpy(s, c->S.data(), sizeof(double) * c->S.size());
	return 0;
}
extern "C" int isg_set_self_rates(isg_ctx *c, const double *s)
{
	HIPCHK(hipSetDevice(c->cfg.device));
	if (ensure_S(c)) return 1;
	memcpy(c->S.data(), s, sizeof(double) * c->S.size());
	HIPCHK(hipMemcpy(c->d_S, c->S.data(), sizeof(double) * c->S.size(), hipMemcpyHostToDevice));
	return 0;
}
extern "C" int isg_get_state(isg_ctx *c, int32_t *s)
{
	HIPCHK(hipSetDevice(c->cfg.device));
	if (ensure_S(c)) return 1;
	memcpy(s, c->state.data(), sizeof(int) * c->state.size());
	return 0;
}
extern "C" int isg_get_indvlkh(isg_ctx *c, double *v)
{
	HIPCHK(hipSetDevice(c->cfg.device));
	if (ensure_lkh(c)) return 1;
	memcpy(v, c->indvlkh.data(), sizeof(double) * c->indvlkh.size());
	return 0;
}
extern "C" int isg_get_alpha(isg_ctx *c, double *a) { *a = c->alpha; return 0; }
extern "C" int isg_set_alpha(isg_ctx *c, double a) { c->alpha = a; return 0; }
extern "C" int isg_get_totallkh(isg_ctx *c, double *t)
{
	HIPCHK(hipSetDevice(c->cfg.device));
	if (ensure_lkh(c)) return 1;
	*t = c->totallkh;
	return 0;
}

extern "C" int isg_ctx_create_poly(const isg_config *cfg, const int32_t *allelenum, const int32_t *seqdata, const int32_t *alleleid, isg_ctx **out)
{
	*out = nullptr;
	if (cfg->P != 4) return fail("isg_ctx_create_poly: ploidy must be 4 (autotetraploid, -ap 1)");
	if (cfg->N < 1 || cfg->L < 1) return fail("isg_ctx_create_poly: empty problem");
	std::vector<int32_t> seq((size_t)cfg->N * cfg->L * 4);
	for (size_t e = 0; e < (size_t)cfg->N * cfg->L; e++)
		for (int k = 0; k < 4; k++) seq[e * 4 + k] = k < alleleid[e] ? seqdata[e * 4 + k] : -1;
	return poly_ctx_create(cfg, allelenum, seq.data(), out);
}
extern "C" int isg_poly_update_geno(isg_ctx *c)
{
	if (!c->poly) return fail("isg_poly_update_geno: not a ploidy 4 context");
	HIPCHK(hipSetDevice(c->cfg.device));
	return poly_geno_sweep(c, 0);
}
extern "C" int isg_get_poly_geno(isg_ctx *c, int32_t *g)
{
	if (!c->poly) return fail("isg_get_poly_geno: not a ploidy 4 context");
	HIPCHK(hipSetDevice(c->cfg.device));
	return poly_get_bytes(c, c->poly->p.geno, g);
}
extern "C" int isg_get_poly_gs(isg_ctx *c, int32_t *gs, int32_t *gcount )
{
	if (!c->poly) return fail("isg_get_poly_gs: not a ploidy 4 context");
	*gs = c->poly->p.GS;
	if (gcount)
		for (int j = 0; j < c->cfg.L; j++) gcount[j] = c->poly->p.allo ? isg_allo_G(c->allelenum[j]) : isg_poly_G(c->allelenum[j]);
	return 0;
}
extern "C" int isg_get_poly_freq2(isg_ctx *c, double *f)
{
	if (!c->poly || !c->poly->p.allo) return fail("isg_get_poly_freq2: not an allotetraploid context");
	if (!c->poly->freq_host) {
		const int L = c->cfg.L, K = c->cfg.K, A = c->Amax, KP = c->poly->p.KP;
		HIPCHK(hipSetDevice(c->cfg.device));
		HIPCHK(hipMemcpyAsync(c->freq_stage.data(), c->poly->p.freq2, sizeof(double) * (size_t)L * A * KP, hipMemcpyDeviceToHost, c->stream));
		HIPCHK(hipStreamSynchronize(c->stream));
		freq_from_device(c->freq_stage.data(), c->poly->freq2_h.data(), K, L, A, KP);
	}
	memcpy(f, c->poly->freq2_h.data(), sizeof(double) * c->poly->freq2_h.size());
	return 0;
}
extern "C" int isg_get_poly_table(isg_ctx *c, int which, float *out)
{
	if (!c->poly) return fail("isg_get_poly_table: not a ploidy 4 context");
	HIPCHK(hipSetDevice(c->cfg.device));
	const PolyDev &p = c->poly->p;
	HIPCHK(hipMemcpyAsync(out, which ? p.genofreq : p.exfreq, sizeof(float) * (size_t)p.K * p.L * p.GS, hipMemcpyDeviceToHost, c->stream));
	HIPCHK(hipStreamSynchronize(c->stream));
	return 0;
}

__device__ __forceinline__ void runmean_dev(double *m, double x, double n, double n1)
{
	const double v = *m;
	*m = (v != 0) ? v * ((n + x / v) / n1) : x / n1;
}
__global__ void k_store_fill(double *p, size_t n, double v)
{
	const size_t i = (size_t)blockIdx.x * blockDim.x + threadIdx.x;
	if (i < n) p[i] = v;
}
__global__ void k_store_chn(const double *qq, double *mqq, double *mqq2, size_t nqq, const double *lkh, double *mlkh, const int *gen, double *mgen,
			    double *mgen2, size_t nind, const double *freq, double *mfreq, double *mfreq2, size_t nfreq, double n, double n1)
{
	const size_t i = (size_t)blockIdx.x * blockDim.x + threadIdx.x;
	if (mqq && i < nqq) {
		const double x = qq[i];
		runmean_dev(&mqq[i], x, n, n1);
		runmean_dev(&mqq2[i], x * x, n, n1);
	}
	if (i < nind) {
		runmean_dev(&mlkh[i], lkh[i], n, n1);
		if (mgen) {
			const int g = gen[i];
			runmean_dev(&mgen[i], (double)g, n, n1);
			runmean_dev(&mgen2[i], (double)(g * g), n, n1);
		}
	}
	if (mfreq && i < nfreq) {
		const double x = freq[i];
		runmean_dev(&mfreq[i], x, n, n1);
		runmean_dev(&mfreq2[i], x * x, n, n1);
	}
}
static void store_free(isg_ctx *c)
{
	for (DevBuf<double> *b : {&c->st_qq, &c->st_qq2, &c->st_lkh, &c->st_gen, &c->st_gen2, &c->st_freq, &c->st_freq2}) b->reset();
	c->st_on = false;
	c->st_step = 0;
}
static int store_alloc_ones(isg_ctx *c, DevBuf<double> *p, size_t n)
{
	HIPCHK(p->alloc(n));
	hipLaunchKernelGGL(k_store_fill, dim3((unsigned)((n + 255) / 256)), dim3(256), 0, c->stream, p->get(), n, 1.0);
	HIPCHK(hipGetLastError());
	return 0;
}
extern "C" int isg_store_begin(isg_ctx *c, int with_freq)
{
	HIPCHK(hipSetDevice(c->cfg.device));
	store_free(c);
	const size_t N = (size_t)c->cfg.N, K = (size_t)c->cfg.K;
	const bool has_qq = c->poly || c->cfg.mode != 0, has_gen = !c->poly && (c->cfg.mode == 2 || c->cfg.mode == 3);
	if (with_freq && c->poly) return fail("isg_store_begin: allele frequencies are only accumulated for ploidy 2 (mcmc.c:1436)");
	if (has_qq && (store_alloc_ones(c, &c->st_qq, N * K) || store_alloc_ones(c, &c->st_qq2, N * K))) return 1;
	if (store_alloc_ones(c, &c->st_lkh, N)) return 1;
	if (has_gen && (store_alloc_ones(c, &c->st_gen, N) || store_alloc_ones(c, &c->st_gen2, N))) return 1;
	if (with_freq) {
		const size_t nf = (size_t)c->cfg.L * c->Amax * c->d.KP;
		if (store_alloc_ones(c, &c->st_freq, nf) || store_alloc_ones(c, &c->st_freq2, nf)) return 1;
	}
	c->st_on = true;
	c->st_step = 0;
	return 0;
}
extern "C" int isg_store_step(isg_ctx *c)
{
	HIPCHK(hipSetDevice(c->cfg.device));
	if (!c->st_on) return fail("isg_store_step: isg_store_begin first");
	if (c->poly && c->poly->freq_host && c->st_freq) return fail("isg_store_step: ploidy 4 keeps no frequency means");
	const size_t N = (size_t)c->cfg.N, K = (size_t)c->cfg.K, nqq = c->st_qq ? N * K : 0, nf = c->st_freq ? (size_t)c->cfg.L * c->Amax * c->d.KP : 0;
	size_t n = nqq > N ? nqq : N;
	if (nf > n) n = nf;
	prof_begin(c);
	hipLaunchKernelGGL(k_store_chn, dim3((unsigned)((n + 255) / 256)), dim3(256), 0, c->stream, (const double *)c->d.qq, c->st_qq, c->st_qq2, nqq,
			   (const double *)c->d.indvlkh, c->st_lkh, (const int *)c->d.gen, c->st_gen, c->st_gen2, N, (const double *)c->d.freq, c->st_freq, c->st_freq2,
			   nf, (double)c->st_step, (double)(1 + c->st_step));
	prof_end(c, "k_store_chn");
	HIPCHK(hipGetLastError());
	c->st_step++;
	return 0;
}
extern "C" int isg_store_fetch(isg_ctx *c, double *qq, double *qq2, double *indvlkh, double *gen, double *gen2, double *freq, double *freq2, long *steps)
{
	HIPCHK(hipSetDevice(c->cfg.device));
	if (!c->st_on) return fail("isg_store_fetch: isg_store_begin first");
	const size_t N = (size_t)c->cfg.N, K = (size_t)c->cfg.K;
	if ((qq || qq2) && !c->st_qq) return fail("isg_store_fetch: this mode keeps no qq means");
	if ((gen || gen2) && !c->st_gen) return fail("isg_store_fetch: this mode keeps no generation means");
	if ((freq || freq2) && !c->st_freq) return fail("isg_store_fetch: isg_store_begin was called without frequencies");
	if (qq) HIPCHK(hipMemcpyAsync(qq, c->st_qq, sizeof(double) * N * K, hipMemcpyDeviceToHost, c->stream));
	if (qq2) HIPCHK(hipMemcpyAsync(qq2, c->st_qq2, sizeof(double) * N * K, hipMemcpyDeviceToHost, c->stream));
	if (indvlkh) HIPCHK(hipMemcpyAsync(indvlkh, c->st_lkh, sizeof(double) * N, hipMemcpyDeviceToHost, c->stream));
	if (gen) HIPCHK(hipMemcpyAsync(gen, c->st_gen, sizeof(double) * N, hipMemcpyDeviceToHost, c->stream));
	if (gen2) HIPCHK(hipMemcpyAsync(gen2, c->st_gen2, sizeof(double) * N, hipMemcpyDeviceToHost, c->stream));
	HIPCHK(hipStreamSynchronize(c->stream));
	for (int which = 0; which < 2; which++) {
		double *dst = which ? freq2 : freq;
		if (!dst) continue;
		const int L = c->cfg.L, A = c->Amax, KP = c->d.KP;
		HIPCHK(hipMemcpyAsync(c->freq_stage.data(), which ? c->st_freq2 : c->st_freq, sizeof(double) * (size_t)L * A * KP, hipMemcpyDeviceToHost, c->stream));
		HIPCHK(hipStreamSynchronize(c->stream));
		freq_from_device(c->freq_stage.data(), dst, (int)K, L, A, KP);
	}
	if (steps) *steps = c->st_step;
	return 0;
}

extern "C" long isg_zq_fallbacks(isg_ctx *c) { return c->zq_fallbacks; }
extern "C" int isg_zq_spec_stats(isg_ctx *c, long out[10])
{
	for (int k = 0; k < 10; k++) out[k] = 0;
	if (!c->zspec) return 0;
	out[0] = c->zspec->sweeps;
	out[1] = c->zspec->done;
	out[2] = c->zspec->lost;
	out[3] = (long)c->zspec->last_probes;
	out[4] = (long)c->zspec->last_fail;
	out[5] = (long)c->zspec->last_rounds;
	out[6] = (long)c->zspec->walk.plan.table_bytes;
	out[7] = (long)c->zspec->walk.plan.seg.size();
	out[8] = (long)c->zspec->lost_fail;
	out[9] = c->zspec->retried;
	return 0;
}
extern "C" int isg_p_device_stats(isg_ctx *c, long out[10])
{
	for (int k = 0; k < 10; k++) out[k] = 0;
	if (!c->pdev) return 0;
	const WalkRun &w = c->pdev->walk;
	out[0] = c->pdev->sweeps - c->pdev->fallbacks;
	out[1] = c->pdev->fallbacks;
	out[2] = (long)w.plan.seg.size();
	out[3] = (long)w.plan.blk.size();
	out[4] = (long)w.plan.table_bytes;
	out[5] = (long)(1000.0 * w.sigma);
	out[6] = (long)(1000.0 * w.scale);
	out[7] = (long)(1000.0 * w.kwin);
	out[8] = c->pdev->retried;
	out[9] = w.fails;
	return 0;
}
extern "C" int isg_profile_enable(isg_ctx *c, int on) { c->prof = on != 0; return 0; }
extern "C" int isg_profile_count(isg_ctx *c) { prof_collect(c); return (int)c->prof_entries.size(); }
extern "C" int isg_profile_get(isg_ctx *c, int idx, char *name, int cap, double *ms, long *n)
{
	if (idx < 0 || idx >= (int)c->prof_entries.size()) return fail("isg_profile_get: index out of range");
	snprintf(name, cap, "%s", c->prof_entries[idx].name.c_str());
	*ms = c->prof_entries[idx].ms;
	*n = c->prof_entries[idx].n;
	return 0;
}
extern "C" int isg_profile_reset(isg_ctx *c) { prof_collect(c); c->prof_entries.clear(); return 0; }

__global__ void __launch_bounds__(256) k_copy16(const uint4 *__restrict__ src, uint4 *__restrict__ dst, size_t n)
{
	const size_t stride = (size_t)gridDim.x * 256;
	for (size_t k = (size_t)blockIdx.x * 256 + threadIdx.x; k < n; k += stride) dst[k] = src[k];
}
extern "C" int isg_copy_bandwidth(int device, size_t bytes, int reps, double *gbs)
{
	*gbs = 0;
	HIPCHK(hipSetDevice(device));
	const size_t n = bytes / 16;
	DevBuf<uint4> a, b;
	HIPCHK(a.alloc(n));
	if (b.alloc(n) != hipSuccess) return fail("isg_copy_bandwidth: out of device memory");
	HIPCHK(hipMemset(a, 1, n * 16));
	hipEvent_t e0, e1;
	HIPCHK(hipEventCreate(&e0));
	HIPCHK(hipEventCreate(&e1));
	int cus = 256;
	(void)hipDeviceGetAttribute(&cus, hipDeviceAttributeMultiprocessorCount, device);
	const dim3 grid((unsigned)(cus * 8));
	for (int w = 0; w < 2; w++) hipLaunchKernelGGL(k_copy16, grid, dim3(256), 0, 0, (const uint4 *)a, b.get(), n);
	HIPCHK(hipEventRecord(e0, 0));
	for (int r = 0; r < reps; r++) hipLaunchKernelGGL(k_copy16, grid, dim3(256), 0, 0, (const uint4 *)a, b.get(), n);
	HIPCHK(hipEventRecord(e1, 0));
	HIPCHK(hipEventSynchronize(e1));
	float ms = 0;
	HIPCHK(hipEventElapsedTime(&ms, e0, e1));
	*gbs = 2.0 * (double)(n * 16) * reps / (ms * 1e-3) / 1e9;
	(void)hipEventDestroy(e0); (void)hipEventDestroy(e1);
	return 0;
}

extern "C" int isg_selftest(void)
{
	static const uint32_t M[3] = {ISG_M1, ISG_M2, ISG_M3}, A[3] = {ISG_A1, ISG_A2, ISG_A3};
	static const double MD[3] = {30269.0, 30307.0, 30323.0};
	for (int g = 0; g < 3; g++) {
		volatile float inv = 1.0f / (float)M[g];
		volatile double md = MD[g];
		const double invd = 1.0 / md;
		for (uint32_t s = 0; s < M[g] + 2000; s++) {
			if (isg_lcg_fast(s, A[g], M[g], inv) != (A[g] * s) % M[g]) return fail("isg_selftest: isg_lcg_fast differs from (a*s) % m");
			if (isg_wh_div(s, md, invd) != (double)s / md) return fail("isg_selftest: isg_wh_div differs from s / m");
		}
	}
	isg_wh_tables tab;
	isg_wh_tables_init(&tab);
	isg_wh s0 = {13, 4, 1972}, s = s0;
	for (uint64_t n = 1; n <= 70000; n++) {
		isg_wh_step(&s);
		if (n % 997 == 0 || n < 600) {
			isg_wh j = isg_wh_jump(&tab, s0, n), j32 = isg_wh_jump32(&tab, s0, (uint32_t)n);
			if (j.s1 != s.s1 || j.s2 != s.s2 || j.s3 != s.s3 || j32.s1 != s.s1 || j32.s2 != s.s2 || j32.s3 != s.s3) return fail("isg_selftest: skip-ahead differs from stepping");
		}
	}
	return 0;
}

#include "isg_rccl.inc"

extern "C" double isg_gelman_rubin(const double *vec, int numchains, int totrep)
{
	const int rep = totrep / numchains;
	std::vector<double> psii(numchains), S(numchains);
	double psi = 0, W = 0, B = 0;
	for (int i = 0; i < numchains; i++) {
		psii[i] = 0;
		for (int j = 0; j < rep; j++) psii[i] += vec[i * rep + j];
		psii[i] = psii[i] / rep;
		psi = psi + psii[i];
	}
	psi = psi / numchains;
	for (int i = 0; i < numchains; i++) {
		S[i] = 0;
		for (int j = 0; j < rep; j++) S[i] += (vec[i * rep + j] - psii[i]) * (vec[i * rep + j] - psii[i]);
		S[i] = S[i] / (rep - 1);
		W += S[i];
	}
	W = W / numchains;
	for (int i = 0; i < numchains; i++) B += (psii[i] - psi) * (psii[i] - psi);
	B = (B * rep) / (numchains - 1);
	double V = (W * (rep - 1)) / rep + B / rep;
	return V / W;
}
```

### instruct_amd/csrc/isg_spec_hip.inc

```
struct SpecProbe {
	int i;
	unsigned x;
	unsigned long long taddr;
};
struct SpecDev {
	unsigned nlist, overflow;
	unsigned nprobes, rounds;
};
struct SpecCtx {
	WalkRun walk;
	int N = 0, K = 0, copies = 2;
	std::vector<int> gam0_h;
	DevBuf<int> d_gam0;
	DevBuf<unsigned long long> d_gpos, d_B, d_offs;
	DevBuf<float> d_alo, d_ahi;
	bool zstrip = false;
	DevBuf<SpecProbe> d_list;
	DevBuf<SpecDev> d_dev;
	DevBuf<ResolveState> d_rs;
	int list_cap = 0, band = 0, rounds = 2;
	float ksig = 4.5f;
	unsigned err_bit = 4u;
	int cooldown = 0;
	int backoff = 0;
	long retried = 0;
	long sweeps = 0, done = 0, lost = 0;
	unsigned last_probes = 0, last_fail = 0, last_rounds = 0, lost_fail = 0;
	int test_abort = 0;
};

typedef float zx_f2 __attribute__((ext_vector_type(2)));
template <int KMAX, int MI>
__global__ void __launch_bounds__(256) k_zexpect(DevView d, double alpha, float ksig, float *alo, float *ahi)
{
	constexpr int KH = (KMAX + 1) / 2, Q4 = (KMAX + 3) / 4;
	__shared__ float red[MI][4][2 * KMAX];
	const int i0 = blockIdx.x * MI, t = threadIdx.x, K = d.K, lane = (int)lane_id();
	zx_f2 qf[MI][KH], lam[MI][KH], var[MI][KH];
#pragma unroll
	for (int m = 0; m < MI; m++)
#pragma unroll
		for (int h = 0; h < KH; h++) {
			const int i = (i0 + m < d.N) ? i0 + m : d.N - 1;
			qf[m][h].x = (2 * h < K) ? (float)d.qq[(size_t)i * K + 2 * h] : 0.f;
			qf[m][h].y = (2 * h + 1 < K) ? (float)d.qq[(size_t)i * K + 2 * h + 1] : 0.f;
			lam[m][h] = (zx_f2)(0.f);
			var[m][h] = (zx_f2)(0.f);
		}
	const unsigned short *grow = (const unsigned short *)(d.geno + (size_t)i0 * d.Lp * 2);
	const bool two = (d.Amax == 2);
	for (int j = t; j < d.Lp; j += 256) {
		float4 B0[Q4], B1[Q4];
		if (two) {
			const float4 *src = (const float4 *)(d.freqf + (size_t)j * 2 * d.KPF);
#pragma unroll
			for (int q = 0; q < Q4; q++) {
				B0[q] = (4 * q < d.KPF) ? src[q] : make_float4(0.f, 0.f, 0.f, 0.f);
				B1[q] = (4 * q < d.KPF) ? src[d.KPF / 4 + q] : make_float4(0.f, 0.f, 0.f, 0.f);
			}
		}
		unsigned gs[MI];
#pragma unroll
		for (int m = 0; m < MI; m++) gs[m] = (i0 + m < d.N) ? grow[(size_t)m * d.Lp + j] : 0xffffu;
#pragma unroll
		for (int m = 0; m < MI; m++) {
			const unsigned g = gs[m];
			const unsigned a0 = g & 0xff, a1 = g >> 8;
			if (a0 == 0xff) continue;
#pragma unroll
			for (int cp = 0; cp < 2; cp++) {
				const unsigned al = cp ? a1 : a0;
				const float *F = d.freqf + ((size_t)j * d.Amax + al) * d.KPF;
				zx_f2 w[KH], tot2 = (zx_f2)(0.f);
#pragma unroll
				for (int q = 0; q < Q4; q++) {
					float4 f = make_float4(0.f, 0.f, 0.f, 0.f);
					if (4 * q < K) {
						if (two) {
							const float4 r0 = B0[q], r1 = B1[q];
							f = al ? r1 : r0;
						} else {
							f = *(const float4 *)(F + 4 * q);
						}
					}
					w[2 * q] = qf[m][2 * q] * (zx_f2){f.x, f.y};
					if (2 * q + 1 < KH) w[2 * q + 1] = qf[m][2 * q + 1] * (zx_f2){f.z, f.w};
				}
#pragma unroll
				for (int h = 0; h < KH; h++) tot2 += w[h];
				const float tot = tot2.x + tot2.y;
				const float inv = (tot > 0.f) ? 1.0f / tot : 0.f;
				const zx_f2 inv2 = (zx_f2)(inv), one2 = (zx_f2)(1.0f);
#pragma unroll
				for (int h = 0; h < KH; h++) {
					const zx_f2 pr = w[h] * inv2;
					lam[m][h] += pr;
					var[m][h] += pr * (one2 - pr);
				}
			}
		}
	}
#pragma unroll
	for (int m = 0; m < MI; m++)
#pragma unroll
		for (int k = 0; k < KMAX; k++) {
			float l = (k & 1) ? lam[m][k / 2].y : lam[m][k / 2].x, v = (k & 1) ? var[m][k / 2].y : var[m][k / 2].x;
#pragma unroll
			for (int o = 32; o > 0; o >>= 1) {
				l += __shfl_down(l, o, 64);
				v += __shfl_down(v, o, 64);
			}
			if (lane == 0) {
				red[m][t >> 6][k] = l;
				red[m][t >> 6][KMAX + k] = v;
			}
		}
	__syncthreads();
	for (int e = t; e < MI * K; e += 256) {
		const int m = e / K, k = e - m * K, i = i0 + m;
		if (i >= d.N) break;
		const float l = red[m][0][k] + red[m][1][k] + red[m][2][k] + red[m][3][k];
		float v = red[m][0][KMAX + k] + red[m][1][KMAX + k] + red[m][2][KMAX + k] + red[m][3][KMAX + k];
		v = v > 0.f ? v : 0.f;
		const float h = ksig * __builtin_sqrtf(v) + 1.0f + 1e-5f * l;
		float lo = __builtin_floorf(l - h), hi = __builtin_ceilf(l + h);
		const float tot = 2.0f * (float)d.nvalid[i];
		if (lo < 0.f) lo = 0.f;
		if (hi > tot) hi = tot;
		if (d.nvalid[i] == 0) lo = hi = 0.f;
		alo[(size_t)i * K + k] = (float)((double)lo + alpha);
		ahi[(size_t)i * K + k] = (float)((double)hi + alpha);
	}
}

__global__ void __launch_bounds__(256) k_zs_band(const WkBlock *blk, const WkSeg *segs, int nseg, const unsigned char *table, const WkState *st, const unsigned long long *T, int N, int band,
						 SpecProbe *list, int cap, SpecDev *dev)
{
	const long id = (long)blockIdx.x * 256 + threadIdx.x;
	const int span = 2 * band + 1;
	const int i = (int)(id / span), j = (int)(id - (long)i * span) - band;
	if (i >= N || st->fail) return;
	int s = 0;
	while (s + 1 < nseg && i >= segs[s].g1) s++;
	const WkSeg S = segs[s];
	const WkBlock B = blk[S.b0 + (i - S.g0) / S.bg];
	const long long x = (long long)T[i] + j;
	const long long col = x - (long long)st->xin[s] - B.wlo;
	if (x < 0 || col < 0 || col >= B.W) return;
	const unsigned long long addr = B.toff + (unsigned long long)(i - B.g0) * (unsigned long long)B.W + (unsigned long long)col;
	const unsigned v = table[addr];
	if (v == WK_IRR || !(v & WK_UFLAG)) return;
	const unsigned slot = atomicAdd(&dev->nlist, 1u);
	if (slot < (unsigned)cap) {
		list[slot].i = i;
		list[slot].x = (unsigned)x;
		list[slot].taddr = addr;
	} else {
		dev->overflow = 1u;
	}
}

#define ISG_ZX_WCH 16
__global__ void __launch_bounds__(256) k_zexpect_w(DevView d, double alpha, float ksig, float *alo, float *ahi)
{
	__shared__ float qs[ISG_KWIDE];
	__shared__ float red[4][2 * ISG_ZX_WCH];
	const int i = blockIdx.x, k0 = blockIdx.y * ISG_ZX_WCH, t = threadIdx.x, K = d.K, lane = (int)lane_id();
	if (t < K) qs[t] = (float)d.qq[(size_t)i * K + t];
	__syncthreads();
	float lam[ISG_ZX_WCH], var[ISG_ZX_WCH];
#pragma unroll
	for (int h = 0; h < ISG_ZX_WCH; h++) lam[h] = var[h] = 0.f;
	const unsigned short *grow = (const unsigned short *)(d.geno + (size_t)i * d.Lp * 2);
	for (int j = t; j < d.Lp; j += 256) {
		const unsigned g = grow[j];
		const unsigned a0 = g & 0xff, a1 = g >> 8;
		if (a0 == 0xff) continue;
		for (int cp = 0; cp < 2; cp++) {
			const float *F = d.freqf + ((size_t)j * d.Amax + (cp ? a1 : a0)) * d.KPF;
			float tot = 0.f;
			for (int m = 0; m < K; m++) tot += qs[m] * F[m];
			const float inv = (tot > 0.f) ? 1.0f / tot : 0.f;
#pragma unroll
			for (int h = 0; h < ISG_ZX_WCH; h++) {
				const bool in = (k0 + h < K);
				const int k = in ? k0 + h : 0;
				const float pr = in ? qs[k] * F[k] * inv : 0.f;
				lam[h] += pr;
				var[h] += pr * (1.0f - pr);
			}
		}
	}
#pragma unroll
	for (int h = 0; h < ISG_ZX_WCH; h++) {
		float l = lam[h], v = var[h];
#pragma unroll
		for (int o = 32; o > 0; o >>= 1) {
			l += __shfl_down(l, o, 64);
			v += __shfl_down(v, o, 64);
		}
		if (lane == 0) {
			red[t >> 6][h] = l;
			red[t >> 6][ISG_ZX_WCH + h] = v;
		}
	}
	__syncthreads();
	const int k = k0 + t;
	if (t < ISG_ZX_WCH && k < K) {
		const float l = red[0][t] + red[1][t] + red[2][t] + red[3][t];
		float v = red[0][ISG_ZX_WCH + t] + red[1][ISG_ZX_WCH + t] + red[2][ISG_ZX_WCH + t] + red[3][ISG_ZX_WCH + t];
		v = v > 0.f ? v : 0.f;
		const float h = ksig * __builtin_sqrtf(v) + 1.0f + 1e-5f * l;
		float lo = __builtin_floorf(l - h), hi = __builtin_ceilf(l + h);
		const float tot = 2.0f * (float)d.nvalid[i];
		if (lo < 0.f) lo = 0.f;
		if (hi > tot) hi = tot;
		if (d.nvalid[i] == 0) lo = hi = 0.f;
		alo[(size_t)i * K + k] = (float)((double)lo + alpha);
		ahi[(size_t)i * K + k] = (float)((double)hi + alpha);
	}
}

template <int BLOCK, int KMAX>
__global__ void __launch_bounds__(BLOCK) k_zq_probe(DevView d, isg_wh base, double alpha, const unsigned long long *Bpre, const SpecProbe *list, SpecDev *dev, int cap, unsigned char *table)
{
	__shared__ ZqSh<KMAX> sh;
	const int t = threadIdx.x;
	{
		const uint16_t *src = (const uint16_t *)d.tab;
		uint16_t *dst = (uint16_t *)&sh.tab;
		for (int k = t; k < (int)(sizeof(isg_wh_tables) / 2); k += BLOCK) dst[k] = src[k];
	}
	__syncthreads();
	const isg_wh mult0 = isg_wh_power(&sh.tab, 8u * (unsigned)t);
	const isg_wh mult_pass = isg_wh_power(&sh.tab, 8u * (unsigned)BLOCK);
	const unsigned n = dev->nlist < (unsigned)cap ? dev->nlist : (unsigned)cap;
	if (blockIdx.x == 0 && t == 0 && n) { dev->nprobes += n; dev->rounds += 1u; }
	for (unsigned p = blockIdx.x; p < n; p += gridDim.x) {
		if (t < 2 * ZqSh<KMAX>::KC) (&sh.hist[0][0])[t] = 0;
		__syncthreads();
		const int i = list[p].i;
		const unsigned long long o = Bpre[i] + 2ull * list[p].x;
		const isg_wh cur = isg_wh_jump(&sh.tab, base, o);
		ZqPrefetch<KMAX> pf;
		zq_prefetch<KMAX>(d, i, 0, pf);
		const unsigned used = zq_one<BLOCK, KMAX, false, false>(d, sh, i, cur, 0, 0, alpha, mult0, mult_pass, pf);
		if (t == 0) {
			const unsigned minimal = 2u * (unsigned)d.nvalid[i] + 2u * (unsigned)d.K;
			unsigned char v = (unsigned char)WK_IRR;
			if (used >= minimal && !((used - minimal) & 1u) && (used - minimal) / 2u <= 126u) v = (unsigned char)((used - minimal) / 2u);
			table[list[p].taddr] = v;
		}
		__syncthreads();
	}
}

__global__ void __launch_bounds__(256) k_zs_offs(const unsigned long long *T, const unsigned long long *Bpre, int N, const WkState *st, const SpecDev *dev, unsigned long long *offs, ResolveState *rs)
{
	const int i = blockIdx.x * 256 + threadIdx.x;
	const bool bad = st->fail != 0u || dev->overflow != 0u || dev->nlist != 0u;
	if (i <= N) offs[i] = bad ? 0ull : Bpre[i] + 2ull * T[i];
	if (i == 0) {
		rs->fail = bad ? 1u : 0u;
		rs->total = bad ? 0ull : Bpre[N] + 2ull * T[N];
		rs->done = 1u;
	}
}

static int spec_create(isg_ctx *c, SpecCtx **out, const std::vector<int> &nvalid, int copies)
{
	*out = nullptr;
	if (!env_flag(getenv("INSTRUCT_ZQ_SPEC_RESOLVE"), true)) return 0;
	const int N = c->cfg.N, K = c->cfg.K;
	if (K > WK_NGMAX) return 0;
	SpecCtx *sp = new SpecCtx();
	sp->N = N;
	sp->K = K;
	sp->copies = copies;
	sp->gam0_h.resize((size_t)N + 1);
	std::vector<unsigned long long> B((size_t)N + 1, 0), gpos((size_t)N * K + 1, 0);
	for (int i = 0; i < N; i++) {
		sp->gam0_h[i] = i * K;
		B[i + 1] = B[i] + (unsigned long long)copies * (unsigned)nvalid[i] + 2ull * (unsigned)K;
		for (int m = 0; m < K; m++) gpos[(size_t)i * K + m] = B[i] + (unsigned long long)copies * (unsigned)nvalid[i] + 2ull * (unsigned)m;
	}
	sp->gam0_h[N] = N * K;
	gpos[(size_t)N * K] = B[N];
	sp->band = (int)env_int(getenv("INSTRUCT_ZQ_SPEC_BAND"), sp->band, 0, 512);
	sp->rounds = (int)env_int(getenv("INSTRUCT_ZQ_SPEC_ROUNDS"), sp->rounds, 0, 16);
	sp->ksig = (float)env_double(getenv("INSTRUCT_ZQ_SPEC_KSIG"), sp->ksig, 1.0);
	sp->walk.seg_groups = (int)env_int(getenv("INSTRUCT_ZQ_SPEC_SEG"), 16384, 64, INT_MAX);
	sp->walk.kwin = env_double(getenv("INSTRUCT_WALK_K"), sp->walk.kwin, 1.0);
	sp->test_abort = (int)env_int(getenv("INSTRUCT_ZQ_SPEC_TEST_ABORT"), 0);
	sp->list_cap = 6 * N + 1024;
	*out = sp;
	HIPCHK(sp->d_gam0.alloc((size_t)N + 1));
	HIPCHK(sp->d_gpos.alloc((size_t)N * K + 1));
	HIPCHK(sp->d_B.alloc((size_t)N + 1));
	HIPCHK(sp->d_offs.alloc((size_t)N + 1));
	HIPCHK(sp->d_alo.alloc((size_t)N * K));
	HIPCHK(sp->d_ahi.alloc((size_t)N * K));
	sp->zstrip = env_flag(getenv("INSTRUCT_ZEXPECT_STRIP"), false);
	HIPCHK(sp->d_list.alloc((size_t)sp->list_cap));
	HIPCHK(sp->d_dev.alloc(1));
	HIPCHK(sp->d_rs.alloc(1));
	HIPCHK(hipMemcpy(sp->d_gam0, sp->gam0_h.data(), sizeof(int) * ((size_t)N + 1), hipMemcpyHostToDevice));
	HIPCHK(hipMemcpy(sp->d_gpos, gpos.data(), sizeof(unsigned long long) * gpos.size(), hipMemcpyHostToDevice));
	HIPCHK(hipMemcpy(sp->d_B, B.data(), sizeof(unsigned long long) * B.size(), hipMemcpyHostToDevice));
	return 0;
}

template <class LE, class LP, class LA>
static int spec_update_ZQ_once(isg_ctx *c, SpecCtx *sp, isg_wh base, bool *done, LE launch_expect, LP launch_probe, LA launch_at, bool second, bool *again)
{
	*done = false;
	*again = false;
	if (!sp) return 0;
	if (!second && sp->cooldown > 0) { sp->cooldown--; return 0; }
	const int N = sp->N, K = sp->K;
	WalkRun &w = sp->walk;
	bool ok = false;
	if (walk_prepare(c, w, sp->gam0_h.data(), N, WK_MODE_INTERVAL, false, &ok, 160)) return 1;
	if (!ok) { sp->cooldown = 1 << 30; return 0; }
	if (!second) sp->sweeps++;
	HIPCHK(hipMemsetAsync(w.d_st, 0, sizeof(WkState), c->stream));
	HIPCHK(hipMemsetAsync(sp->d_dev, 0, sizeof(SpecDev), c->stream));
	HIPCHK(hipMemsetAsync(sp->d_rs, 0, sizeof(ResolveState), c->stream));
	HIPCHK(hipMemcpyAsync(c->d_qqsave, c->d.qq, sizeof(double) * (size_t)N * K, hipMemcpyDeviceToDevice, c->stream));
	prof_begin(c);
	launch_expect(sp->d_alo, sp->d_ahi);
	prof_end(c, "k_zexpect");
	WalkInputs in;
	in.gam0 = sp->d_gam0; in.gpos = sp->d_gpos; in.gcnt = nullptr; in.alo = sp->d_alo; in.ahi = sp->d_ahi; in.base = base;
	const int nseg = (int)w.plan.seg.size();
	walk_launch_centers(c, w, in, "k_wk_centers_Z");
	for (int s = 0; s < nseg; s++) {
		walk_launch_tables(c, w, in, s, "k_wk_table_Z");
		walk_launch_walk(c, w, in, s, 0, 0, "k_wk_walk_Z");
	}
	auto list_on_path = [&]() {
		(void)hipMemsetAsync(sp->d_dev, 0, 2 * sizeof(unsigned), c->stream);
		const long nthr = (long)N * (2 * sp->band + 1);
		prof_begin(c);
		hipLaunchKernelGGL(k_zs_band, dim3((unsigned)((nthr + 255) / 256)), dim3(256), 0, c->stream, (const WkBlock *)w.d_blk, (const WkSeg *)w.d_seg, nseg, (const unsigned char *)w.d_table,
				   (const WkState *)w.d_st, (const unsigned long long *)w.d_T, N, sp->band, sp->d_list, sp->list_cap, sp->d_dev);
		prof_end(c, "k_zs_band");
	};
	auto round = [&]() {
		prof_begin(c);
		launch_probe(1024);
		prof_end(c, "k_zq_probe");
		(void)hipMemsetAsync((char *)w.d_st.get() + offsetof(WkState, sum_d), 0, sizeof(WkState) - offsetof(WkState, sum_d), c->stream);
		for (int s = 0; s < nseg; s++) walk_launch_walk(c, w, in, s, 0, 1, "k_wk_walk_Z");
		list_on_path();
	};
	auto finish = [&]() {
		prof_begin(c);
		hipLaunchKernelGGL(k_zs_offs, dim3((unsigned)((N + 1 + 255) / 256)), dim3(256), 0, c->stream, (const unsigned long long *)w.d_T, (const unsigned long long *)sp->d_B, N, (const WkState *)w.d_st,
				   (const SpecDev *)sp->d_dev, sp->d_offs, sp->d_rs);
		prof_end(c, "k_zs_offs");
		prof_begin(c);
		launch_at();
		prof_end(c, "k_zq_at");
	};
	list_on_path();
	for (int r = 0; r < sp->rounds; r++) round();
	finish();
	HIPCHK(hipGetLastError());
	struct { unsigned done, fail; unsigned long long total; } hr;
	WkState hs;
	SpecDev hd;
	unsigned err[4] = {0, 0, 0, 0};
	HIPCHK(hipMemcpyAsync(&hr, &sp->d_rs.get()->done, sizeof(hr), hipMemcpyDeviceToHost, c->stream));
	HIPCHK(hipMemcpyAsync(&hs, w.d_st, sizeof(hs), hipMemcpyDeviceToHost, c->stream));
	HIPCHK(hipMemcpyAsync(&hd, sp->d_dev, sizeof(hd), hipMemcpyDeviceToHost, c->stream));
	HIPCHK(hipMemcpyAsync(err, c->d_err, sizeof(err), hipMemcpyDeviceToHost, c->stream));
	HIPCHK(hipStreamSynchronize(c->stream));
	for (int extra = 0; extra < 12 && !hs.fail && !hd.overflow && hd.nlist != 0u; extra++) {
		round();
		finish();
		HIPCHK(hipGetLastError());
		HIPCHK(hipMemcpyAsync(&hr, &sp->d_rs.get()->done, sizeof(hr), hipMemcpyDeviceToHost, c->stream));
		HIPCHK(hipMemcpyAsync(&hs, w.d_st, sizeof(hs), hipMemcpyDeviceToHost, c->stream));
		HIPCHK(hipMemcpyAsync(&hd, sp->d_dev, sizeof(hd), hipMemcpyDeviceToHost, c->stream));
		HIPCHK(hipMemcpyAsync(err, c->d_err, sizeof(err), hipMemcpyDeviceToHost, c->stream));
		HIPCHK(hipStreamSynchronize(c->stream));
	}
	sp->last_probes = hd.nprobes;
	sp->last_rounds = hd.rounds;
	sp->last_fail = hs.fail | (hd.overflow ? 16u : 0u) | ((err[0] & sp->err_bit) ? 32u : 0u) | (hd.nlist ? 64u : 0u);
	bool good = hr.done && !hr.fail && !(err[0] & sp->err_bit);
	if (sp->test_abort > 0 && --sp->test_abort == 0) good = false;
	walk_adapt(w, hs);
	if (!good) {
		if (err[0] & sp->err_bit) {
			err[0] &= ~sp->err_bit;
			HIPCHK(hipMemcpyAsync(c->d_err, err, sizeof(unsigned), hipMemcpyHostToDevice, c->stream));
		}
		HIPCHK(hipMemcpyAsync(c->d.qq, c->d_qqsave, sizeof(double) * (size_t)N * K, hipMemcpyDeviceToDevice, c->stream));
		HIPCHK(hipStreamSynchronize(c->stream));
		sp->lost_fail |= sp->last_fail;
		if (!second && (hs.fail & 1u) && !(hs.fail & ~1u)) {
			*again = true;
			return 0;
		}
		sp->lost++;
		sp->cooldown = sp->backoff;
		sp->backoff = sp->backoff ? (sp->backoff < 64 ? sp->backoff * 2 : 64) : 1;
		return 0;
	}
	if (hd.nprobes > (unsigned)(2 * N)) sp->cooldown = 2;
	sp->backoff = 0;
	sp->done++;
	host_advance(c, hr.total);
	c->h_qq = false;
	*done = true;
	return 0;
}

template <class LE, class LP, class LA>
static int spec_update_ZQ_with(isg_ctx *c, SpecCtx *sp, isg_wh base, bool *done, LE launch_expect, LP launch_probe, LA launch_at)
{
	bool again = false;
	if (spec_update_ZQ_once(c, sp, base, done, launch_expect, launch_probe, launch_at, false, &again)) return 1;
	if (!again) return 0;
	sp->retried++;
	return spec_update_ZQ_once(c, sp, base, done, launch_expect, launch_probe, launch_at, true, &again);
}

template <int KMAX>
static void spec_launch_expect(isg_ctx *c, SpecCtx *sp, float *alo, float *ahi)
{
	if constexpr (KMAX > ISG_KCAP) {
		hipLaunchKernelGGL(k_zexpect_w, dim3((unsigned)c->cfg.N, (unsigned)((c->cfg.K + ISG_ZX_WCH - 1) / ISG_ZX_WCH)), dim3(256), 0, c->stream, c->d, c->alpha, sp->ksig, alo, ahi);
	} else {
		constexpr int MI = KMAX <= 8 ? 4 : KMAX <= 16 ? 2 : 1;
		hipLaunchKernelGGL((k_zexpect<KMAX, MI>), dim3((unsigned)((c->cfg.N + MI - 1) / MI)), dim3(256), 0, c->stream, c->d, c->alpha, sp->ksig, alo, ahi);
	}
}
template <int KMAX>
static void spec_launch_probe(isg_ctx *c, SpecCtx *sp, isg_wh base, int grid)
{
	hipLaunchKernelGGL((k_zq_probe<256, KMAX>), dim3(grid), dim3(256), 0, c->stream, c->d, base, c->alpha, (const unsigned long long *)sp->d_B, (const SpecProbe *)sp->d_list,
			   sp->d_dev, sp->list_cap, sp->walk.d_table);
}
template <int KMAX>
static void spec_launch_at(isg_ctx *c, SpecCtx *sp, isg_wh base)
{
	hipLaunchKernelGGL((k_zq_at<256, KMAX>), dim3(c->cfg.N), dim3(256), 0, c->stream, c->d, base, c->alpha, (const ResolveState *)sp->d_rs, (const unsigned long long *)sp->d_offs);
}
static int spec_update_ZQ(isg_ctx *c, SpecCtx *sp, isg_wh base, bool *done)
{
	const int K = c->cfg.K;
	return spec_update_ZQ_with(c, sp, base, done,
				   [&](float *alo, float *ahi) { kdispatch(KL_ZQ(), K, [&](auto km) { spec_launch_expect<decltype(km)::value>(c, sp, alo, ahi); }); },
				   [&](int grid) { kdispatch(KL_ZQ(), K, [&](auto km) { spec_launch_probe<decltype(km)::value>(c, sp, base, grid); }); },
				   [&]() { kdispatch(KL_ZQ(), K, [&](auto km) { spec_launch_at<decltype(km)::value>(c, sp, base); }); });
}
```

### instruct_amd/csrc/isg_walk_hip.inc

```
#include "isg_walk_plan.h"

__global__ void __launch_bounds__(64) k_wk_bpred(WkCenterArgs A)
{
	extern __shared__ __attribute__((aligned(16))) unsigned char wk_lds[];
	wk_bpred_body(A, (int)blockIdx.x, (int)blockDim.x, wk_lds);
}
__global__ void __launch_bounds__(256) k_wk_centers(WkCenterArgs A)
{
	extern __shared__ __attribute__((aligned(16))) unsigned char wk_lds[];
	wk_centers_body(A, (int)blockIdx.x, (int)blockDim.x, wk_lds);
}
template <int MODE>
__global__ void __launch_bounds__(256) k_wk_table(WkTableArgs A, unsigned tab_off)
{
	extern __shared__ __attribute__((aligned(16))) unsigned char wk_lds[];
	{
		const uint16_t *src = (const uint16_t *)A.tab;
		uint16_t *dst = (uint16_t *)(wk_lds + tab_off);
		for (int k = threadIdx.x; k < (int)(sizeof(isg_wh_tables) / 2); k += blockDim.x) dst[k] = src[k];
	}
	__syncthreads();
	A.tab = (const isg_wh_tables *)(wk_lds + tab_off);
	A.mode = MODE;
	wk_table_body(A, (int)blockIdx.x, (int)blockDim.x, wk_lds);
}
__global__ void __launch_bounds__(1024) k_wk_block(WkWalkArgs A)
{
	extern __shared__ __attribute__((aligned(16))) unsigned char wk_lds[];
	wk_block_body(A, (int)blockIdx.x, (int)blockDim.x, wk_lds);
}
__global__ void __launch_bounds__(512) k_wk_compose(WkWalkArgs A)
{
	extern __shared__ __attribute__((aligned(16))) unsigned char wk_lds[];
	wk_compose_body(A, (int)blockIdx.x, (int)blockDim.x, wk_lds);
}
__global__ void __launch_bounds__(512) k_wk_top(WkWalkArgs A)
{
	extern __shared__ __attribute__((aligned(16))) unsigned char wk_lds[];
	wk_top_body(A, (int)blockDim.x, wk_lds);
}
__global__ void __launch_bounds__(256) k_wk_expand(WkWalkArgs A)
{
	extern __shared__ __attribute__((aligned(16))) unsigned char wk_lds[];
	wk_expand_body(A, (int)blockIdx.x, (int)blockDim.x, wk_lds);
}
__global__ void __launch_bounds__(256) k_wk_final(WkWalkArgs A)
{
	extern __shared__ __attribute__((aligned(16))) unsigned char wk_lds[];
	wk_final_body(A, (int)blockIdx.x, (int)blockDim.x, wk_lds);
}

struct WalkRun {
	WkPlan plan;
	bool plan_ok = false, attrs_set = false;
	int mode = WK_MODE_EXACT;
	DevBuf<WkBlock> d_blk;
	DevBuf<WkSuper> d_sup;
	DevBuf<WkSeg> d_seg;
	DevBuf<int> d_hw, d_ent_sup, d_ent_blk;
	DevBuf<float> d_bpred;
	DevBuf<unsigned char> d_table;
	DevBuf<unsigned short> d_maps;
	DevBuf<unsigned long long> d_T;
	DevBuf<WkState> d_st;
	double sigma = 1.0, kwin = 4.0, rho_hi = 0.8;
	double kwin0 = 0.0;
	hvec<unsigned char> stage;
	int clean = 0;
	float scale = 1.0f;
	int seg_groups = 8192;
	int plan_seg_groups = 0, plan_slack = 0;
	long runs = 0, fails = 0;
};

static int walk_prepare(isg_ctx *c, WalkRun &w, const int *gam0_h, int G, int mode, bool reuse, bool *ok, int entry_slack = 0)
{
	*ok = false;
	if (w.plan_ok && w.mode == mode && w.plan.groups == G && w.plan.rho_hi == w.rho_hi && w.plan.sigma == w.sigma && w.plan.kwin == w.kwin && w.plan.reuse == reuse &&
	    w.plan_seg_groups == w.seg_groups && w.plan_slack == entry_slack) {
		*ok = true;
		return 0;
	}
	WkPlan np;
	if (!wk_plan_build(np, gam0_h, G, w.rho_hi, w.sigma, w.kwin, w.seg_groups, reuse, mode, entry_slack)) { w.plan_ok = false; return 0; }
	w.plan_seg_groups = w.seg_groups;
	w.plan_slack = entry_slack;
	const bool same = w.plan_ok && np.blk.size() == w.plan.blk.size() && np.sup.size() == w.plan.sup.size() && np.seg.size() == w.plan.seg.size() &&
			  memcmp(np.blk.data(), w.plan.blk.data(), sizeof(WkBlock) * np.blk.size()) == 0 && memcmp(np.hw.data(), w.plan.hw.data(), sizeof(int) * np.hw.size()) == 0;
	w.mode = mode;
	if (!same) {
		HIPCHK(hipStreamSynchronize(c->stream));
		w.plan = np;
		HIPCHK(w.d_blk.grow(np.blk.size()));
		HIPCHK(w.d_hw.grow(np.blk.size()));
		HIPCHK(w.d_ent_blk.grow(np.blk.size()));
		HIPCHK(w.d_bpred.grow(np.blk.size()));
		HIPCHK(w.d_sup.grow(np.sup.size()));
		HIPCHK(w.d_ent_sup.grow(np.sup.size()));
		HIPCHK(w.d_table.grow(np.table_bytes + 64));
		HIPCHK(w.d_maps.grow(np.maps_elems + 64));
		HIPCHK(w.d_T.grow((size_t)G + 1));
		if (!w.d_st) HIPCHK(w.d_st.alloc(1));
		if (!w.d_seg) HIPCHK(w.d_seg.alloc(WK_MAXSEG));
		{
			const size_t b0 = sizeof(WkSeg) * np.seg.size(), b1 = sizeof(WkBlock) * np.blk.size(), b2 = sizeof(WkSuper) * np.sup.size(), b3 = sizeof(int) * np.hw.size();
			const size_t o1 = (b0 + 63) & ~(size_t)63, o2 = o1 + ((b1 + 63) & ~(size_t)63), o3 = o2 + ((b2 + 63) & ~(size_t)63);
			w.stage.resize(o3 + b3 + 64);
			memcpy(w.stage.data(), w.plan.seg.data(), b0);
			memcpy(w.stage.data() + o1, w.plan.blk.data(), b1);
			memcpy(w.stage.data() + o2, w.plan.sup.data(), b2);
			memcpy(w.stage.data() + o3, w.plan.hw.data(), b3);
			HIPCHK(hipMemcpyAsync(w.d_seg, w.stage.data(), b0, hipMemcpyHostToDevice, c->stream));
			HIPCHK(hipMemcpyAsync(w.d_blk, w.stage.data() + o1, b1, hipMemcpyHostToDevice, c->stream));
			HIPCHK(hipMemcpyAsync(w.d_sup, w.stage.data() + o2, b2, hipMemcpyHostToDevice, c->stream));
			HIPCHK(hipMemcpyAsync(w.d_hw, w.stage.data() + o3, b3, hipMemcpyHostToDevice, c->stream));
			HIPCHK(hipStreamSynchronize(c->stream));
		}
		w.plan_ok = true;
	} else {
		w.plan.sigma = np.sigma;
		w.plan.kwin = np.kwin;
		w.plan.rho_hi = np.rho_hi;
	}
	if (!w.attrs_set) {
		HIPCHK(hipFuncSetAttribute((const void *)k_wk_table<WK_MODE_EXACT>, hipFuncAttributeMaxDynamicSharedMemorySize, 160 * 1024));
		HIPCHK(hipFuncSetAttribute((const void *)k_wk_table<WK_MODE_INTERVAL>, hipFuncAttributeMaxDynamicSharedMemorySize, 160 * 1024));
		HIPCHK(hipFuncSetAttribute((const void *)k_wk_block, hipFuncAttributeMaxDynamicSharedMemorySize, 160 * 1024));
		HIPCHK(hipFuncSetAttribute((const void *)k_wk_compose, hipFuncAttributeMaxDynamicSharedMemorySize, 160 * 1024));
		HIPCHK(hipFuncSetAttribute((const void *)k_wk_top, hipFuncAttributeMaxDynamicSharedMemorySize, 160 * 1024));
		HIPCHK(hipFuncSetAttribute((const void *)k_wk_expand, hipFuncAttributeMaxDynamicSharedMemorySize, 160 * 1024));
		w.attrs_set = true;
	}
	*ok = true;
	return 0;
}

struct WalkInputs {
	const int *gam0;
	const unsigned long long *gpos;
	const int *gcnt;
	const float *alo, *ahi;
	isg_wh base;
	const float *tape = nullptr;
	unsigned long long tape_len = 0;
};
static void walk_launch_centers(isg_ctx *c, WalkRun &w, const WalkInputs &in, const char *pname)
{
	WkCenterArgs C;
	C.blk = w.d_blk; C.hw = w.d_hw; C.bpred = w.d_bpred; C.st = w.d_st; C.gam0 = in.gam0; C.gcnt = in.gcnt; C.alo = in.alo; C.ahi = in.ahi; C.seg = w.plan.seg[0]; C.segs = w.d_seg;
	C.mode = w.mode; C.scale = w.scale;
	int nbmax = 0;
	for (const WkSeg &S : w.plan.seg) nbmax = S.nb > nbmax ? S.nb : nbmax;
	prof_begin(c);
	hipLaunchKernelGGL(k_wk_bpred, dim3((unsigned)w.plan.blk.size()), dim3(64), sizeof(float) * 64, c->stream, C);
	hipLaunchKernelGGL(k_wk_centers, dim3((unsigned)w.plan.seg.size()), dim3(256), sizeof(float) * (size_t)nbmax, c->stream, C);
	prof_end(c, pname);
}
static void walk_launch_tables(isg_ctx *c, WalkRun &w, const WalkInputs &in, int s, const char *pname)
{
	const WkSeg S = w.plan.seg[s];
	WkTableArgs A;
	A.blk = w.d_blk; A.gam0 = in.gam0; A.gpos = in.gpos; A.gcnt = in.gcnt; A.alo = in.alo; A.ahi = in.ahi; A.table = w.d_table; A.st = w.d_st; A.base = in.base; A.tab = c->d.tab; A.tape = in.tape; A.tape_len = in.tape_len;
	A.seg_b0 = S.b0; A.seg_g0 = S.g0; A.bg = S.bg; A.seg = s; A.mode = w.mode;
	const unsigned tab_off = (unsigned)((w.plan.lds_table + 15) & ~(size_t)15);
	prof_begin(c);
	if (w.mode == WK_MODE_INTERVAL) hipLaunchKernelGGL(k_wk_table<WK_MODE_INTERVAL>, dim3((unsigned)(S.g1 - S.g0)), dim3(256), tab_off + sizeof(isg_wh_tables), c->stream, A, tab_off);
	else hipLaunchKernelGGL(k_wk_table<WK_MODE_EXACT>, dim3((unsigned)(S.g1 - S.g0)), dim3(256), tab_off + sizeof(isg_wh_tables), c->stream, A, tab_off);
	prof_end(c, pname);
}
static void walk_launch_walk(isg_ctx *c, WalkRun &w, const WalkInputs &in, int s, int strict, int keep_origin, const char *pname)
{
	const WkSeg S = w.plan.seg[s];
	WkWalkArgs A;
	A.blk = w.d_blk; A.sup = w.d_sup; A.table = w.d_table; A.maps = w.d_maps; A.ent_sup = w.d_ent_sup; A.ent_blk = w.d_ent_blk; A.T = w.d_T; A.st = w.d_st;
	A.seg = S; A.segno = s; A.mode = w.mode; A.strict = strict; A.keep_origin = keep_origin; A.total_groups = w.plan.groups; A.bpred = w.d_bpred; A.gam0 = in.gam0; A.scale = w.scale;
	prof_begin(c);
	hipLaunchKernelGGL(k_wk_block, dim3((unsigned)S.nb), dim3(1024), w.plan.lds_block, c->stream, A);
	hipLaunchKernelGGL(k_wk_compose, dim3((unsigned)S.ns), dim3(512), w.plan.lds_compose, c->stream, A);
	hipLaunchKernelGGL(k_wk_top, dim3(1), dim3(512), w.plan.lds_top, c->stream, A);
	hipLaunchKernelGGL(k_wk_expand, dim3((unsigned)S.ns), dim3(256), w.plan.lds_compose, c->stream, A);
	hipLaunchKernelGGL(k_wk_final, dim3((unsigned)S.nb), dim3(256), (size_t)WK_BG * WK_STRIP, c->stream, A);
	prof_end(c, pname);
}
static void walk_adapt(WalkRun &w, const WkState &hs)
{
	w.runs++;
	if (w.kwin0 == 0.0) w.kwin0 = w.kwin;
	if (hs.fail) {
		w.fails++;
		if ((hs.fail & 1u) && w.kwin < 12.0) {
			w.kwin *= 1.25;
			w.clean = 0;
		}
		return;
	}
	if (++w.clean >= 512 && w.kwin > w.kwin0) {
		w.kwin = (w.kwin / 1.25 > w.kwin0) ? w.kwin / 1.25 : w.kwin0;
		w.clean = 0;
	}
	if (hs.pred > 0.0 && hs.nblk > 0) {
		const double sc = (double)hs.sum_d / hs.pred;
		if (sc > 0.5 && sc < 2.0) w.scale = (float)(0.7 * w.scale + 0.3 * sc);
	}
	if (hs.ngam > 64.0) {
		const double var = hs.resid2 / hs.ngam;
		double sg = sqrt(var > 0.25 ? var : 0.25);
		if (sg > 3.0) sg = 3.0;
		sg = ceil((0.5 * w.sigma + 0.5 * sg) * 20.0) / 20.0;
		if (sg < 0.9) sg = 0.9;
		w.sigma = sg;
	}
}

struct PDevCtx {
	WalkRun walk;
	int G = 0, NG = 0;
	std::vector<int> gam0_h;
	DevBuf<int> d_gam0;
	DevBuf<int> d_gidx;
	DevBuf<int> d_gcnt;
	DevBuf<unsigned long long> d_gpos;
	DevBuf<unsigned> d_part;
	DevBuf<float> d_tapef;
	unsigned long long tape_len = 0;
	bool usable = false;
	long sweeps = 0, fallbacks = 0, retried = 0;
};

__global__ void __launch_bounds__(256) k_pd_gather(const int *cnt, const int *gidx, int ng, int *gcnt, unsigned *part)
{
	__shared__ unsigned red[4];
	const int k0 = ((int)blockIdx.x * 256 + (int)threadIdx.x) * 4;
	unsigned s = 0;
#pragma unroll
	for (int q = 0; q < 4; q++) {
		if (k0 + q < ng) {
			const int v = cnt[gidx[k0 + q]];
			gcnt[k0 + q] = v;
			s += v == 0 ? 1u : 2u;
		}
	}
	s = wave_sum_u32(s);
	if (lane_id() == 0) red[threadIdx.x >> 6] = s;
	__syncthreads();
	if (threadIdx.x == 0) part[blockIdx.x] = red[0] + red[1] + red[2] + red[3];
}
__global__ void __launch_bounds__(256) k_pd_scan(const int *gcnt, int ng, const unsigned *part, unsigned long long *gpos)
{
	__shared__ unsigned long long red[4];
	__shared__ unsigned sm[256 / 64 + 1];
	const int t = threadIdx.x;
	unsigned long long b = 0;
	for (int k = t; k < (int)blockIdx.x; k += 256) b += part[k];
#pragma unroll
	for (int o = 32; o > 0; o >>= 1) b += __shfl_down(b, o, 64);
	if (lane_id() == 0) red[t >> 6] = b;
	__syncthreads();
	const unsigned long long base = red[0] + red[1] + red[2] + red[3];
	const int k0 = ((int)blockIdx.x * 256 + t) * 4;
	unsigned u[4], s = 0;
#pragma unroll
	for (int q = 0; q < 4; q++) {
		u[q] = (k0 + q < ng) ? (gcnt[k0 + q] == 0 ? 1u : 2u) : 0u;
		s += u[q];
	}
	unsigned tot;
	unsigned pre = block_excl_scan<256>(s, sm, &tot);
#pragma unroll
	for (int q = 0; q < 4; q++) {
		if (k0 + q < ng) gpos[k0 + q] = base + pre;
		pre += u[q];
	}
	if (k0 <= ng && ng < k0 + 4) gpos[ng] = base + pre;
}

__global__ void __launch_bounds__(128) k_pdirich_at(DevView d, isg_wh base, const int *gam0, const int *gidx, const int *gcnt, const unsigned long long *gpos,
						     const unsigned long long *T, int G, WkState *st)
{
	const int g = blockIdx.x * blockDim.x + threadIdx.x;
	if (g >= G || st->fail) return;
	const int g0 = gam0[g], n = gam0[g + 1] - g0;
	const unsigned long long p = gpos[g0] + 2ull * T[g], p1 = gpos[g0 + n] + 2ull * T[g + 1];
	isg_cursor c;
	c.s = isg_wh_jump(d.tab, base, p);
	c.used = 0;
	c.tape = nullptr;
	double sum = 0;
	for (int a = 0; a < n; a++) {
		const double v = isg_rgamma(&c, (double)gcnt[g0 + a] + 1.0);
		const int ix = gidx[g0 + a], row = ix / d.K, k = ix - row * d.K;
		d.freq[(size_t)row * d.KP + k] = v;
		sum += v;
	}
	for (int a = 0; a < n; a++) {
		const int ix = gidx[g0 + a], row = ix / d.K, k = ix - row * d.K;
		d.freq[(size_t)row * d.KP + k] /= sum;
	}
	if ((unsigned long long)c.used != p1 - p) atomicOr(&st->fail, 8u);
}

static int pdev_create(isg_ctx *c, PDevCtx **out, int L, int K, int Amax, const int *allelenum, int min_alleles)
{
	*out = nullptr;
	if (!env_flag(getenv("INSTRUCT_P_DEVICE"), true)) return 0;
	PDevCtx *p = new PDevCtx();
	std::vector<int> gidx;
	p->gam0_h.push_back(0);
	for (int k = 0; k < K; k++)
		for (int j = 0; j < L; j++) {
			const int Aj = allelenum[j];
			if (Aj <= min_alleles) continue;
			if (Aj > WK_NGMAX) { delete p; return 0; }
			for (int a = 0; a < Aj; a++) gidx.push_back((j * Amax + a) * K + k);
			p->gam0_h.push_back((int)gidx.size());
		}
	p->G = (int)p->gam0_h.size() - 1;
	p->NG = (int)gidx.size();
	if (p->G < 1) { delete p; return 0; }
	p->walk.seg_groups = (int)env_int(getenv("INSTRUCT_WALK_SEG"), 12800, 64, INT_MAX);
	p->walk.kwin = env_double(getenv("INSTRUCT_WALK_K"), p->walk.kwin, 1.0);
	*out = p;
	HIPCHK(p->d_gam0.alloc((size_t)p->G + 1));
	HIPCHK(p->d_gidx.alloc(p->NG));
	HIPCHK(p->d_gcnt.alloc(p->NG));
	HIPCHK(p->d_gpos.alloc((size_t)p->NG + 1));
	HIPCHK(p->d_part.alloc((size_t)(p->NG + 1023) / 1024 + 2));
	p->tape_len = 2ull * (unsigned long long)p->NG + (unsigned long long)(1.7 * p->NG) + (unsigned long long)(12.0 * sqrt((double)p->NG)) + 8192ull;
	HIPCHK(p->d_tapef.alloc(p->tape_len));
	HIPCHK(hipMemcpy(p->d_gam0, p->gam0_h.data(), sizeof(int) * (p->G + 1), hipMemcpyHostToDevice));
	HIPCHK(hipMemcpy(p->d_gidx, gidx.data(), sizeof(int) * p->NG, hipMemcpyHostToDevice));
	p->usable = true;
	return 0;
}

static int pdev_update_P_once(isg_ctx *c, PDevCtx *p, bool *done, bool second, bool *again)
{
	*done = false;
	*again = false;
	if (!p || !p->usable) return 0;
	bool ok = false;
	if (walk_prepare(c, p->walk, p->gam0_h.data(), p->G, WK_MODE_EXACT, true, &ok)) return 1;
	if (!ok) { p->usable = false; return 0; }
	WalkRun &w = p->walk;
	HIPCHK(hipMemsetAsync(w.d_st, 0, sizeof(WkState), c->stream));
	prof_begin(c);
	{
		const unsigned nchunk = (unsigned)((p->NG + 1023) / 1024) + 1u;
		hipLaunchKernelGGL(k_pd_gather, dim3(nchunk), dim3(256), 0, c->stream, (const int *)c->d.cnt, (const int *)p->d_gidx, p->NG, p->d_gcnt, p->d_part);
		hipLaunchKernelGGL(k_pd_scan, dim3(nchunk), dim3(256), 0, c->stream, (const int *)p->d_gcnt, p->NG, (const unsigned *)p->d_part, p->d_gpos);
	}
	prof_end(c, "k_pd_prep");
	prof_begin(c);
	hipLaunchKernelGGL(k_tapef, dim3((unsigned)((p->tape_len + 2047) / 2048)), dim3(256), 0, c->stream, c->d.tab, c->rng, (unsigned long long)p->tape_len, p->d_tapef);
	prof_end(c, "k_tapef_P");
	WalkInputs in;
	in.gam0 = p->d_gam0; in.gpos = p->d_gpos; in.gcnt = p->d_gcnt; in.alo = nullptr; in.ahi = nullptr; in.base = c->rng;
	in.tape = p->d_tapef; in.tape_len = p->tape_len;
	walk_launch_centers(c, w, in, "k_wk_centers_P");
	for (int s = 0; s < (int)w.plan.seg.size(); s++) {
		walk_launch_tables(c, w, in, s, "k_wk_table_P");
		walk_launch_walk(c, w, in, s, 0, 0, "k_wk_walk_P");
	}
	prof_begin(c);
	hipLaunchKernelGGL(k_pdirich_at, dim3((unsigned)((p->G + 127) / 128)), dim3(128), 0, c->stream, c->d, c->rng, (const int *)p->d_gam0, (const int *)p->d_gidx, (const int *)p->d_gcnt,
			   (const unsigned long long *)p->d_gpos, (const unsigned long long *)w.d_T, p->G, w.d_st);
	prof_end(c, "k_pdirich_at");
	HIPCHK(hipGetLastError());
	WkState hs;
	unsigned long long tail[2] = {0, 0};
	HIPCHK(hipMemcpyAsync(&hs, w.d_st, sizeof(hs), hipMemcpyDeviceToHost, c->stream));
	HIPCHK(hipMemcpyAsync(&tail[0], p->d_gpos + p->NG, sizeof(unsigned long long), hipMemcpyDeviceToHost, c->stream));
	HIPCHK(hipMemcpyAsync(&tail[1], w.d_T + p->G, sizeof(unsigned long long), hipMemcpyDeviceToHost, c->stream));
	HIPCHK(hipStreamSynchronize(c->stream));
	walk_adapt(w, hs);
	if (!second && hs.fail == 1u) {
		*again = true;
		return 0;
	}
	p->sweeps++;
	if (hs.fail) {
		p->fallbacks++;
		return 0;
	}
	host_advance(c, tail[0] + 2ull * tail[1]);
	*done = true;
	return 0;
}
static int pdev_update_P(isg_ctx *c, PDevCtx *p, bool *done)
{
	bool again = false;
	if (pdev_update_P_once(c, p, done, false, &again)) return 1;
	if (!again) return 0;
	p->retried++;
	return pdev_update_P_once(c, p, done, true, &again);
}
```

Before: 341.6 iterations/s.

## Enqueue next-stage GPU work before host readback syncs to hide round-trip latency

Replaces hipStreamSynchronize readbacks with pinned mailbox copies plus events, and before waiting on each event it enqueues follow-on GPU work. That work is refresh_freqf in update_P, the ZQ expectation prologue in update_G, the loglik sweep in update_ZQ, and the lkh total and counts prep in update_alpha. A validity bitmask tracks which of this ahead work can be reused, and settle() calls guard the public accessors. The aim is to keep the GPU busy while the host waits on small readbacks. The cost is considerable state-tracking complexity and a risk of stale reuse if any invalidation is missed.

```diff
diff --git a/instruct_amd/csrc/isg_ahead.h b/instruct_amd/csrc/isg_ahead.h
--- /dev/null
+++ b/instruct_amd/csrc/isg_ahead.h
@@ -0,0 +1,55 @@
+#ifndef ISG_AHEAD_H
+#define ISG_AHEAD_H
+
+enum {
+	AH_FREQF = 1u << 0,
+	AH_EXPECT = 1u << 1,
+	AH_LKH = 1u << 2,
+	AH_LKH_TOTAL = 1u << 3,
+	AH_COUNTS = 1u << 4,
+	AH_ALL = (1u << 5) - 1u
+};
+enum { AH_LOOK_P, AH_LOOK_G, AH_LOOK_ZQ, AH_LOOK_ALPHA, AH_NLOOKS };
+
+struct AheadState {
+	unsigned have;
+	unsigned pending;
+};
+
+static inline void ahead_init(AheadState *s) { s->have = 0u; s->pending = 0u; }
+static inline bool ahead_has(const AheadState *s, unsigned item) { return (s->have & item) == item; }
+static inline void ahead_clear(AheadState *s, unsigned items)
+{
+	if (items & AH_LKH) items |= AH_LKH_TOTAL;
+	s->have &= ~items;
+}
+static inline void ahead_set(AheadState *s, unsigned item)
+{
+	if ((item & AH_LKH_TOTAL) && !((s->have | item) & AH_LKH)) item &= ~(unsigned)AH_LKH_TOTAL;
+	s->have |= item & AH_ALL;
+}
+static inline bool ahead_take(AheadState *s, unsigned item)
+{
+	const bool had = ahead_has(s, item);
+	ahead_clear(s, item);
+	return had;
+}
+
+static inline void ahead_wrote_z(AheadState *s) { ahead_clear(s, AH_COUNTS | AH_LKH); }
+static inline void ahead_wrote_freq(AheadState *s) { ahead_clear(s, AH_FREQF | AH_EXPECT | AH_LKH); }
+static inline void ahead_wrote_qq(AheadState *s) { ahead_clear(s, AH_EXPECT | AH_LKH); }
+static inline void ahead_wrote_gen(AheadState *s) { ahead_clear(s, AH_LKH); }
+static inline void ahead_wrote_alpha(AheadState *s) { ahead_clear(s, AH_EXPECT); }
+static inline void ahead_chain_init(AheadState *s) { ahead_clear(s, AH_ALL); }
+static inline void ahead_end_iteration(AheadState *s) { ahead_clear(s, AH_ALL & ~(unsigned)AH_COUNTS); }
+
+static inline void ahead_look_recorded(AheadState *s, int look) { s->pending |= 1u << look; }
+static inline void ahead_look_waited(AheadState *s, int look) { s->pending &= ~(1u << look); }
+static inline unsigned ahead_settle(AheadState *s)
+{
+	const unsigned m = s->pending;
+	s->pending = 0u;
+	return m;
+}
+
+#endif
diff --git a/instruct_amd/csrc/isg_hip.hip b/instruct_amd/csrc/isg_hip.hip
--- a/instruct_amd/csrc/isg_hip.hip
+++ b/instruct_amd/csrc/isg_hip.hip
@@ -19,6 +19,7 @@
 #include "isg_host_dirichlet.h"
 #include "isg_kdispatch.h"
 #include "isg_devbuf.h"
+#include "isg_ahead.h"
 
 #define ISG_KCAP 32
 #define ISG_KWIDE 64
@@ -123,6 +124,8 @@
 	PinnedBuf<double> htape;
 	DevEvent ev_tape;
 	DevEvent ev_cnt;
+	PinnedBuf<unsigned char> mail;
+	DevEvent ev_look[AH_NLOOKS];
 	DevBuf<double> st_qq, st_qq2, st_lkh, st_gen, st_gen2, st_freq, st_freq2;
 };
 struct isg_ctx : CtxBufs {
@@ -173,7 +176,10 @@
 	int spop_tree = 1;
 	int test_abort = 0;
 	long zq_fallbacks = 0;
-	hvec<double> ratios_h;
+	AheadState ah;
+	bool lookahead = true;
+	bool la_on = false;
+	bool zq_pro_ready = false;
 	bool h_qq, h_gen, h_S, h_lkh;
 	long st_step = 0;
 	bool st_on = false;
@@ -1740,6 +1746,29 @@
 	if (ptr && bytes && hipHostRegister(ptr, bytes, hipHostRegisterDefault) == hipSuccess) c->pinned.push_back(ptr);
 	else (void)hipGetLastError();
 }
+enum { MAIL_P = 0, MAIL_G = 2048, MAIL_ZQ = 2560, MAIL_RATIOS = 4096 };
+struct MailG { uint64_t used; unsigned err[4]; };
+template <class T> static T *mail_slot(isg_ctx *c, size_t off) { return (T *)(c->mail.get() + off); }
+static int look_record(isg_ctx *c, int look)
+{
+	if (!c->ev_look[look]) HIPCHK(hipEventCreateWithFlags(&c->ev_look[look].e, hipEventDisableTiming));
+	HIPCHK(hipEventRecord(c->ev_look[look], c->stream));
+	ahead_look_recorded(&c->ah, look);
+	return 0;
+}
+static int look_wait(isg_ctx *c, int look)
+{
+	HIPCHK(hipEventSynchronize(c->ev_look[look]));
+	ahead_look_waited(&c->ah, look);
+	return 0;
+}
+static int settle(isg_ctx *c)
+{
+	const unsigned m = ahead_settle(&c->ah);
+	for (int l = 0; m && l < AH_NLOOKS; l++)
+		if (m & (1u << l)) HIPCHK(hipEventSynchronize(c->ev_look[l]));
+	return 0;
+}
 #define HOST_T(c, k, t0) do { if ((c)->host_timing) { const auto t1_ = std::chrono::steady_clock::now(); (c)->host_t[k] += std::chrono::duration<double>(t1_ - (t0)).count(); (t0) = t1_; } } while (0)
 enum { HOSTP_REQUEST = 1, HOSTP_DRAW = 2 };
 struct HostPSecond { const int *d_cnt; int *cnt_h; double *freq_h; };
@@ -1794,6 +1823,10 @@
 }
 static std::atomic<int> g_live_ctx[64];
 static void ctx_count(isg_ctx *c, int delta);
+static int launch_lkh_sweep(isg_ctx *c);
+static void launch_lkh_total(isg_ctx *c);
+static int lkh_total_ahead(isg_ctx *c);
+static bool lkh_sweep_is_generic(const isg_ctx *c);
 #include "isg_resolve_hip.inc"
 #include "isg_walk_hip.inc"
 #include "isg_spec_hip.inc"
@@ -1847,6 +1880,10 @@
 	c->prof = false;
 	c->host_timing = env_flag(getenv("INSTRUCT_HOST_TIMING"), false);
 	c->host_tape = env_flag(getenv("INSTRUCT_HOST_TAPE"), true);
+	c->lookahead = env_flag(getenv("INSTRUCT_LOOKAHEAD"), true);
+	ahead_init(&c->ah);
+	HIPCHK(c->mail.alloc(MAIL_RATIOS + (c->cfg.P == 2 ? sizeof(double) * (size_t)N * K : 0)));
+	memset(c->mail.get(), 0, MAIL_RATIOS);
 	c->h_qq = c->h_gen = c->h_S = c->h_lkh = true;
 	isg_wh_tables_init(&c->tab_h);
 	HIPCHK(c->d_tab.upload(&c->tab_h, 1));
@@ -1977,7 +2014,6 @@
 	HIPCHK(c->d_state.alloc_zero(ISG_KWIDE));
 	HIPCHK(c->d_ratios.alloc_zero((size_t)N * K));
 	HIPCHK(c->d_total.alloc_zero(1));
-	c->ratios_h.assign((size_t)N * K, 0.0);
 	keyed_layout(c);
 	if (cfg->mode == 0 && !d.lftab) return fail("isg_ctx_create: mode 0 needs its log frequency table (INSTRUCT_LL_TABLES must not be 0)");
 	if (cfg->mode == 4) {
@@ -1999,6 +2035,7 @@
 }
 extern "C" int isg_get_seeds(isg_ctx *c, long s[3])
 {
+	if (settle(c)) return 1;
 	if (c->raw_valid) { s[0] = c->raw_seed[0]; s[1] = c->raw_seed[1]; s[2] = c->raw_seed[2]; }
 	else { s[0] = c->rng.s1; s[1] = c->rng.s2; s[2] = c->rng.s3; }
 	return 0;
@@ -2041,6 +2078,7 @@
 }
 static int download_freq(isg_ctx *c)
 {
+	if (settle(c)) return 1;
 	const int L = c->cfg.L, K = c->cfg.K, A = c->Amax, KP = c->d.KP;
 	HIPCHK(hipMemcpyAsync(c->freq_stage.data(), c->d.freq, sizeof(double) * (size_t)L * A * KP, hipMemcpyDeviceToHost, c->stream));
 	HIPCHK(hipStreamSynchronize(c->stream));
@@ -2049,6 +2087,7 @@
 }
 static int ensure_qq(isg_ctx *c)
 {
+	if (settle(c)) return 1;
 	if (c->h_qq) return 0;
 	HIPCHK(hipMemcpyAsync(c->qq.data(), c->d.qq, sizeof(double) * c->qq.size(), hipMemcpyDeviceToHost, c->stream));
 	HIPCHK(hipMemcpyAsync(c->qqnum.data(), c->d.qqnum, sizeof(int) * c->qqnum.size(), hipMemcpyDeviceToHost, c->stream));
@@ -2058,6 +2097,7 @@
 }
 static int ensure_gen(isg_ctx *c)
 {
+	if (settle(c)) return 1;
 	if (c->h_gen) return 0;
 	HIPCHK(hipMemcpyAsync(c->gen.data(), c->d.gen, sizeof(int) * c->gen.size(), hipMemcpyDeviceToHost, c->stream));
 	HIPCHK(hipStreamSynchronize(c->stream));
@@ -2066,6 +2106,7 @@
 }
 static int ensure_S(isg_ctx *c)
 {
+	if (settle(c)) return 1;
 	if (c->h_S) return 0;
 	HIPCHK(hipMemcpyAsync(c->S.data(), c->d_S, sizeof(double) * c->S.size(), hipMemcpyDeviceToHost, c->stream));
 	HIPCHK(hipMemcpyAsync(c->state.data(), c->d_state, sizeof(int) * c->cfg.K, hipMemcpyDeviceToHost, c->stream));
@@ -2075,6 +2116,7 @@
 }
 static int ensure_lkh(isg_ctx *c)
 {
+	if (settle(c)) return 1;
 	if (c->h_lkh) return 0;
 	unsigned e[4] = {0, 0, 0, 0};
 	HIPCHK(hipMemcpyAsync(c->indvlkh.data(), c->d.indvlkh, sizeof(double) * c->indvlkh.size(), hipMemcpyDeviceToHost, c->stream));
@@ -2138,19 +2180,34 @@
 	c->ahead_valid = false;
 	if (c->poly || is_keyed(c) || !c->host_tape) return 0;
 	if (c->pdev && c->pdev->usable) return 0;
+	if (ahead_has(&c->ah, AH_COUNTS)) return 0;
 	if (launch_count(c)) return 1;
 	return host_update_P(c, HOSTP_REQUEST, c->d.cnt, nullptr, true);
 }
+static int counts_ahead(isg_ctx *c)
+{
+	if (!c->la_on || c->poly) return 0;
+	const bool dev = c->pdev && c->pdev->usable;
+	if (!is_keyed(c) && !dev) return 0;
+	if (launch_count(c)) return 1;
+	if (!is_keyed(c)) pdev_launch_prep(c, c->pdev);
+	HIPCHK(hipGetLastError());
+	ahead_set(&c->ah, AH_COUNTS);
+	return 0;
+}
 
 extern "C" int isg_update_P(isg_ctx *c)
 {
 	HIPCHK(hipSetDevice(c->cfg.device));
 	if (c->poly) return poly_update_P(c);
+	if (settle(c)) return 1;
 	DevView &d = c->d;
 	const int L = c->cfg.L, K = c->cfg.K;
 	const bool ahead = c->ahead_valid && !is_keyed(c) && c->ahead_rng.s1 == c->rng.s1 && c->ahead_rng.s2 == c->rng.s2 && c->ahead_rng.s3 == c->rng.s3;
 	c->ahead_valid = false;
-	if (!ahead && launch_count(c)) return 1;
+	const bool counted = ahead_take(&c->ah, AH_COUNTS);
+	ahead_wrote_freq(&c->ah);
+	if (!ahead && !counted && launch_count(c)) return 1;
 	if (is_keyed(c)) {
 		int n = K * L, B = 256;
 		prof_begin(c);
@@ -2161,8 +2218,8 @@
 	}
 	if (!ahead && c->pdev && c->pdev->usable) {
 		bool done = false;
-		if (pdev_update_P(c, c->pdev, &done)) return 1;
-		if (done) return refresh_freqf(c);
+		if (pdev_update_P(c, c->pdev, &done, counted)) return 1;
+		if (done) return ahead_take(&c->ah, AH_FREQF) ? 0 : refresh_freqf(c);
 	}
 	if (host_update_P(c, ahead ? HOSTP_DRAW : HOSTP_REQUEST | HOSTP_DRAW, d.cnt, nullptr, true)) return 1;
 	auto ht0 = std::chrono::steady_clock::now();
@@ -2181,6 +2238,7 @@
 	if (c->cfg.mode != 2) return 0;
 	HIPCHK(hipSetDevice(c->cfg.device));
 	if (c->poly) return poly_update_S_POP(c);
+	if (settle(c)) return 1;
 	const int K = c->cfg.K;
 	isg_wh start = is_keyed(c) ? isg_wh_jump(&c->tab_h, c->origin, iter_base(c) + c->ky[KY_OFFS]) : c->rng;
 	if (c->cfg.back_refl == 1 && K <= ISG_SPOP_TREE_K && c->spop_tree) {
@@ -2215,6 +2273,8 @@
 	NOT_POLY(c, "isg_update_G");
 	if (c->cfg.mode != 2 && c->cfg.mode != 3) return 0;
 	HIPCHK(hipSetDevice(c->cfg.device));
+	if (settle(c)) return 1;
+	ahead_wrote_gen(&c->ah);
 	DevView &d = c->d;
 	double *d_S = c->d_S;
 	isg_wh base = is_keyed(c) ? isg_wh_jump(&c->tab_h, c->origin, iter_base(c) + c->ky[KY_OFFG]) : c->rng;
@@ -2231,13 +2291,14 @@
 	HIPCHK(hipGetLastError());
 	c->h_gen = false;
 	if (!is_keyed(c)) {
-		uint64_t used = 0;
-		unsigned e[4] = {0, 0, 0, 0};
-		HIPCHK(hipMemcpyAsync(&used, c->d_pos, sizeof(used), hipMemcpyDeviceToHost, c->stream));
-		HIPCHK(hipMemcpyAsync(e, c->d_err, sizeof(e), hipMemcpyDeviceToHost, c->stream));
-		HIPCHK(hipStreamSynchronize(c->stream));
-		if (report_dev_err(e)) return 1;
-		host_advance(c, used);
+		MailG *m = mail_slot<MailG>(c, MAIL_G);
+		HIPCHK(hipMemcpyAsync(&m->used, c->d_pos, sizeof(m->used), hipMemcpyDeviceToHost, c->stream));
+		HIPCHK(hipMemcpyAsync(m->err, c->d_err, sizeof(m->err), hipMemcpyDeviceToHost, c->stream));
+		if (look_record(c, AH_LOOK_G)) return 1;
+		if (c->la_on && c->zspec && spec_ZQ_prologue_ahead(c, c->zspec)) return 1;
+		if (look_wait(c, AH_LOOK_G)) return 1;
+		if (report_dev_err(m->err)) return 1;
+		host_advance(c, m->used);
 	}
 	return 0;
 }
@@ -2299,6 +2360,10 @@
 	c->ahead_valid = false;
 	HIPCHK(hipSetDevice(c->cfg.device));
 	if (c->poly) return poly_update_ZQ(c, init_flag);
+	if (settle(c)) return 1;
+	const bool prologue = ahead_take(&c->ah, AH_EXPECT) && !init_flag;
+	ahead_wrote_z(&c->ah);
+	ahead_wrote_qq(&c->ah);
 	const int K = c->cfg.K;
 	bool chain = !is_keyed(c);
 	isg_wh base = chain ? c->rng : c->origin;
@@ -2308,7 +2373,7 @@
 	c->d.tape_len = 0;
 	if (chain && !init_flag && c->zspec) {
 		bool done = false;
-		if (spec_update_ZQ(c, c->zspec, base, &done)) return 1;
+		if (spec_update_ZQ(c, c->zspec, base, &done, prologue)) return 1;
 		if (done) return 0;
 	}
 	if (chain && !init_flag && c->rs) {
@@ -2380,6 +2445,7 @@
 {
 	NOT_POLY(c, "isg_update_alpha");
 	HIPCHK(hipSetDevice(c->cfg.device));
+	if (settle(c)) return 1;
 	const size_t NK = (size_t)c->cfg.N * c->cfg.K;
 	if (is_keyed(c)) host_seek(c, iter_base(c) + c->ky[KY_OFFA]);
 	isg_cursor cur;
@@ -2394,13 +2460,17 @@
 		hipLaunchKernelGGL(k_alpha_ratios, dim3((unsigned)((NK + 255) / 256)), dim3(256), 0, c->stream, c->d, ralpha, c->alpha, c->d_ratios);
 		prof_end(c, "k_alpha_ratios");
 		HIPCHK(hipGetLastError());
-		HIPCHK(hipMemcpyAsync(c->ratios_h.data(), c->d_ratios, sizeof(double) * NK, hipMemcpyDeviceToHost, c->stream));
-		HIPCHK(hipStreamSynchronize(c->stream));
+		double *ratios_h = mail_slot<double>(c, MAIL_RATIOS);
+		HIPCHK(hipMemcpyAsync(ratios_h, c->d_ratios, sizeof(double) * NK, hipMemcpyDeviceToHost, c->stream));
+		if (look_record(c, AH_LOOK_ALPHA)) return 1;
+		if (lkh_total_ahead(c) || counts_ahead(c)) return 1;
+		if (look_wait(c, AH_LOOK_ALPHA)) return 1;
 		double mh = 1.0;
-		for (size_t k = 0; k < NK; k++) mh *= c->ratios_h[k];
+		for (size_t k = 0; k < NK; k++) mh *= ratios_h[k];
 		double thr = (1 > mh) ? mh : 1;
 		c->alpha = (host_next(c) < thr) ? ralpha : c->alpha;
-	}
+	} else if (lkh_total_ahead(c) || counts_ahead(c)) return 1;
+	ahead_wrote_alpha(&c->ah);
 	return update_P_ahead(c);
 }
 
@@ -2411,6 +2481,18 @@
 	if (c->cfg.mode == 0) return noadm_cal_lkh(c);
 	if (c->cfg.mode == 4) return inbreed_cal_lkh(c);
 	if (c->cfg.mode == 5) return indiv_cal_lkh_F(c);
+	if (settle(c)) return 1;
+	const bool total = ahead_has(&c->ah, AH_LKH_TOTAL);
+	const bool swept = ahead_take(&c->ah, AH_LKH);
+	if (!swept && launch_lkh_sweep(c)) return 1;
+	if (!swept || !total) launch_lkh_total(c);
+	HIPCHK(hipGetLastError());
+	c->h_lkh = false;
+	return 0;
+}
+static bool lkh_sweep_is_generic(const isg_ctx *c) { return !c->poly && c->cfg.mode != 0 && c->cfg.mode != 4 && c->cfg.mode != 5; }
+static int launch_lkh_sweep(isg_ctx *c)
+{
 	DevView &d = c->d;
 	prof_begin(c);
 	if (d.lli && d.mode == 2) hipLaunchKernelGGL((k_loglik_int<256, false>), dim3(d.N), dim3(256), 0, c->stream, d);
@@ -2418,11 +2500,21 @@
 	else if (d.K > ISG_KCAP) hipLaunchKernelGGL((k_loglik_w<256, false>), dim3(d.N), dim3(256), 0, c->stream, d);
 	else hipLaunchKernelGGL((k_loglik<256, false>), dim3(d.N), dim3(256), 0, c->stream, d);
 	prof_end(c, "k_loglik_lkh");
+	HIPCHK(hipGetLastError());
+	return 0;
+}
+static void launch_lkh_total(isg_ctx *c)
+{
 	prof_begin(c);
-	hipLaunchKernelGGL(k_lkh_total<1024>, dim3(1), dim3(1024), 0, c->stream, d, c->d_total);
+	hipLaunchKernelGGL(k_lkh_total<1024>, dim3(1), dim3(1024), 0, c->stream, c->d, c->d_total);
 	prof_end(c, "k_lkh_total");
+}
+static int lkh_total_ahead(isg_ctx *c)
+{
+	if (!c->la_on || !ahead_has(&c->ah, AH_LKH)) return 0;
+	launch_lkh_total(c);
 	HIPCHK(hipGetLastError());
-	c->h_lkh = false;
+	ahead_set(&c->ah, AH_LKH_TOTAL);
 	return 0;
 }
 
@@ -2457,6 +2549,8 @@
 	c->ahead_valid = false;
 	if (c->poly || c->cfg.mode != 0) return fail("isg_update_Z: mode 0 (-v 0) only");
 	HIPCHK(hipSetDevice(c->cfg.device));
+	if (settle(c)) return 1;
+	ahead_wrote_z(&c->ah);
 	return noadm_update_Z(c, init_flag);
 }
 
@@ -2474,6 +2568,11 @@
 		HIPCHK(hipSetDevice(c->cfg.device));
 		return poly_iteration(c);
 	}
+	struct LaScope {
+		isg_ctx *c;
+		explicit LaScope(isg_ctx *p) : c(p) { c->la_on = c->lookahead; }
+		~LaScope() { c->la_on = false; ahead_end_iteration(&c->ah); }
+	} la_scope(c);
 	if (isg_update_P(c)) return 1;
 	if (c->cfg.mode == 0) {
 		if (isg_update_Z(c, 0)) return 1;
@@ -2510,6 +2609,8 @@
 	c->ahead_valid = false;
 	HIPCHK(hipSetDevice(c->cfg.device));
 	if (c->poly) return poly_chain_init(c, initd);
+	if (settle(c)) return 1;
+	ahead_chain_init(&c->ah);
 	const int N = c->cfg.N, K = c->cfg.K;
 	c->origin = c->rng;
 	c->iter = 0;
@@ -2589,6 +2690,7 @@
 {
 	HIPCHK(hipSetDevice(c->cfg.device));
 	if (c->poly) return poly_get_bytes(c, c->poly->p.z, z);
+	if (settle(c)) return 1;
 	const int N = c->cfg.N, L = c->cfg.L, Lp = c->d.Lp;
 	std::vector<uint8_t> h((size_t)N * Lp * 2);
 	HIPCHK(hipMemcpyAsync(h.data(), c->d.z, h.size(), hipMemcpyDeviceToHost, c->stream));
@@ -2601,6 +2703,8 @@
 	c->ahead_valid = false;
 	NOT_POLY(c, "isg_set_z");
 	HIPCHK(hipSetDevice(c->cfg.device));
+	if (settle(c)) return 1;
+	ahead_wrote_z(&c->ah);
 	const int N = c->cfg.N, L = c->cfg.L, Lp = c->d.Lp;
 	std::vector<uint8_t> h((size_t)N * Lp * 2, 0xff);
 	for (int i = 0; i < N; i++)
@@ -2624,6 +2728,8 @@
 {
 	NOT_POLY(c, "isg_set_freq");
 	HIPCHK(hipSetDevice(c->cfg.device));
+	if (settle(c)) return 1;
+	ahead_wrote_freq(&c->ah);
 	memcpy(c->freq.data(), f, sizeof(double) * c->freq.size());
 	if (upload_freq(c)) return 1;
 	HIPCHK(hipStreamSynchronize(c->stream));
@@ -2640,6 +2746,7 @@
 {
 	HIPCHK(hipSetDevice(c->cfg.device));
 	if (ensure_qq(c)) return 1;
+	ahead_wrote_qq(&c->ah);
 	memcpy(c->qq.data(), q, sizeof(double) * c->qq.size());
 	HIPCHK(hipMemcpy(c->d.qq, q, sizeof(double) * c->qq.size(), hipMemcpyHostToDevice));
 	return 0;
@@ -2663,6 +2770,8 @@
 {
 	NOT_POLY(c, "isg_set_generation");
 	HIPCHK(hipSetDevice(c->cfg.device));
+	if (settle(c)) return 1;
+	ahead_wrote_gen(&c->ah);
 	memcpy(c->gen.data(), g, sizeof(int) * c->gen.size());
 	HIPCHK(hipMemcpy(c->d.gen, g, sizeof(int) * c->gen.size(), hipMemcpyHostToDevice));
 	c->h_gen = true;
@@ -2697,8 +2806,19 @@
 	memcpy(v, c->indvlkh.data(), sizeof(double) * c->indvlkh.size());
 	return 0;
 }
-extern "C" int isg_get_alpha(isg_ctx *c, double *a) { *a = c->alpha; return 0; }
-extern "C" int isg_set_alpha(isg_ctx *c, double a) { c->alpha = a; return 0; }
+extern "C" int isg_get_alpha(isg_ctx *c, double *a)
+{
+	if (settle(c)) return 1;
+	*a = c->alpha;
+	return 0;
+}
+extern "C" int isg_set_alpha(isg_ctx *c, double a)
+{
+	if (settle(c)) return 1;
+	ahead_wrote_alpha(&c->ah);
+	c->alpha = a;
+	return 0;
+}
 extern "C" int isg_get_totallkh(isg_ctx *c, double *t)
 {
 	HIPCHK(hipSetDevice(c->cfg.device));
diff --git a/instruct_amd/csrc/isg_spec_hip.inc b/instruct_amd/csrc/isg_spec_hip.inc
--- a/instruct_amd/csrc/isg_spec_hip.inc
+++ b/instruct_amd/csrc/isg_spec_hip.inc
@@ -310,12 +310,24 @@
 	return 0;
 }
 
-template <class LE, class LP, class LA>
-static int spec_update_ZQ_once(isg_ctx *c, SpecCtx *sp, isg_wh base, bool *done, LE launch_expect, LP launch_probe, LA launch_at, bool second, bool *again)
-{
-	*done = false;
-	*again = false;
-	if (!sp) return 0;
+struct MailZQ {
+	struct { unsigned done, fail; unsigned long long total; } r;
+	WkState st;
+	SpecDev dev;
+	unsigned err[4];
+};
+static_assert(sizeof(MailZQ) <= MAIL_RATIOS - MAIL_ZQ, "update_ZQ's slot of the mailbox");
+
+static WalkInputs spec_inputs(const SpecCtx *sp, isg_wh base)
+{
+	WalkInputs in;
+	in.gam0 = sp->d_gam0; in.gpos = sp->d_gpos; in.gcnt = nullptr; in.alo = sp->d_alo; in.ahi = sp->d_ahi; in.base = base;
+	return in;
+}
+template <class LE>
+static int spec_ZQ_prologue(isg_ctx *c, SpecCtx *sp, LE launch_expect, bool second, bool *ready)
+{
+	*ready = false;
 	if (!second && sp->cooldown > 0) { sp->cooldown--; return 0; }
 	const int N = sp->N, K = sp->K;
 	WalkRun &w = sp->walk;
@@ -330,10 +342,27 @@
 	prof_begin(c);
 	launch_expect(sp->d_alo, sp->d_ahi);
 	prof_end(c, "k_zexpect");
-	WalkInputs in;
-	in.gam0 = sp->d_gam0; in.gpos = sp->d_gpos; in.gcnt = nullptr; in.alo = sp->d_alo; in.ahi = sp->d_ahi; in.base = base;
+	isg_wh nobase;
+	nobase.s1 = nobase.s2 = nobase.s3 = 0;
+	walk_launch_centers(c, w, spec_inputs(sp, nobase), "k_wk_centers_Z");
+	HIPCHK(hipGetLastError());
+	*ready = true;
+	return 0;
+}
+
+template <class LE, class LP, class LA>
+static int spec_update_ZQ_once(isg_ctx *c, SpecCtx *sp, isg_wh base, bool *done, LE launch_expect, LP launch_probe, LA launch_at, bool second, bool *again, bool pro_done)
+{
+	*done = false;
+	*again = false;
+	if (!sp) return 0;
+	bool ready = pro_done && c->zq_pro_ready;
+	if (!pro_done && spec_ZQ_prologue(c, sp, launch_expect, second, &ready)) return 1;
+	if (!ready) return 0;
+	const int N = sp->N, K = sp->K;
+	WalkRun &w = sp->walk;
+	const WalkInputs in = spec_inputs(sp, base);
 	const int nseg = (int)w.plan.seg.size();
-	walk_launch_centers(c, w, in, "k_wk_centers_Z");
 	for (int s = 0; s < nseg; s++) {
 		walk_launch_tables(c, w, in, s, "k_wk_table_Z");
 		walk_launch_walk(c, w, in, s, 0, 0, "k_wk_walk_Z");
@@ -367,25 +396,32 @@
 	for (int r = 0; r < sp->rounds; r++) round();
 	finish();
 	HIPCHK(hipGetLastError());
-	struct { unsigned done, fail; unsigned long long total; } hr;
-	WkState hs;
-	SpecDev hd;
-	unsigned err[4] = {0, 0, 0, 0};
-	HIPCHK(hipMemcpyAsync(&hr, &sp->d_rs.get()->done, sizeof(hr), hipMemcpyDeviceToHost, c->stream));
-	HIPCHK(hipMemcpyAsync(&hs, w.d_st, sizeof(hs), hipMemcpyDeviceToHost, c->stream));
-	HIPCHK(hipMemcpyAsync(&hd, sp->d_dev, sizeof(hd), hipMemcpyDeviceToHost, c->stream));
-	HIPCHK(hipMemcpyAsync(err, c->d_err, sizeof(err), hipMemcpyDeviceToHost, c->stream));
-	HIPCHK(hipStreamSynchronize(c->stream));
-	for (int extra = 0; extra < 12 && !hs.fail && !hd.overflow && hd.nlist != 0u; extra++) {
+	MailZQ *m = mail_slot<MailZQ>(c, MAIL_ZQ);
+	auto look = [&]() -> int {
+		HIPCHK(hipMemcpyAsync(&m->r, &sp->d_rs.get()->done, sizeof(m->r), hipMemcpyDeviceToHost, c->stream));
+		HIPCHK(hipMemcpyAsync(&m->st, w.d_st, sizeof(m->st), hipMemcpyDeviceToHost, c->stream));
+		HIPCHK(hipMemcpyAsync(&m->dev, sp->d_dev, sizeof(m->dev), hipMemcpyDeviceToHost, c->stream));
+		HIPCHK(hipMemcpyAsync(m->err, c->d_err, sizeof(m->err), hipMemcpyDeviceToHost, c->stream));
+		return look_record(c, AH_LOOK_ZQ);
+	};
+	if (look()) return 1;
+	bool lkh_early = false;
+	if (c->la_on && lkh_sweep_is_generic(c)) {
+		if (launch_lkh_sweep(c)) return 1;
+		lkh_early = true;
+	}
+	if (look_wait(c, AH_LOOK_ZQ)) return 1;
+	for (int extra = 0; extra < 12 && !m->st.fail && !m->dev.overflow && m->dev.nlist != 0u; extra++) {
+		lkh_early = false;
 		round();
 		finish();
 		HIPCHK(hipGetLastError());
-		HIPCHK(hipMemcpyAsync(&hr, &sp->d_rs.get()->done, sizeof(hr), hipMemcpyDeviceToHost, c->stream));
-		HIPCHK(hipMemcpyAsync(&hs, w.d_st, sizeof(hs), hipMemcpyDeviceToHost, c->stream));
-		HIPCHK(hipMemcpyAsync(&hd, sp->d_dev, sizeof(hd), hipMemcpyDeviceToHost, c->stream));
-		HIPCHK(hipMemcpyAsync(err, c->d_err, sizeof(err), hipMemcpyDeviceToHost, c->stream));
-		HIPCHK(hipStreamSynchronize(c->stream));
-	}
+		if (look() || look_wait(c, AH_LOOK_ZQ)) return 1;
+	}
+	const auto hr = m->r;
+	const WkState hs = m->st;
+	const SpecDev hd = m->dev;
+	unsigned err[4] = {m->err[0], m->err[1], m->err[2], m->err[3]};
 	sp->last_probes = hd.nprobes;
 	sp->last_rounds = hd.rounds;
 	sp->last_fail = hs.fail | (hd.overflow ? 16u : 0u) | ((err[0] & sp->err_bit) ? 32u : 0u) | (hd.nlist ? 64u : 0u);
@@ -414,18 +450,19 @@
 	sp->done++;
 	host_advance(c, hr.total);
 	c->h_qq = false;
+	if (lkh_early) ahead_set(&c->ah, AH_LKH);
 	*done = true;
 	return 0;
 }
 
 template <class LE, class LP, class LA>
-static int spec_update_ZQ_with(isg_ctx *c, SpecCtx *sp, isg_wh base, bool *done, LE launch_expect, LP launch_probe, LA launch_at)
+static int spec_update_ZQ_with(isg_ctx *c, SpecCtx *sp, isg_wh base, bool *done, LE launch_expect, LP launch_probe, LA launch_at, bool pro_done = false)
 {
 	bool again = false;
-	if (spec_update_ZQ_once(c, sp, base, done, launch_expect, launch_probe, launch_at, false, &again)) return 1;
+	if (spec_update_ZQ_once(c, sp, base, done, launch_expect, launch_probe, launch_at, false, &again, pro_done)) return 1;
 	if (!again) return 0;
 	sp->retried++;
-	return spec_update_ZQ_once(c, sp, base, done, launch_expect, launch_probe, launch_at, true, &again);
+	return spec_update_ZQ_once(c, sp, base, done, launch_expect, launch_probe, launch_at, true, &again, false);
 }
 
 template <int KMAX>
@@ -449,11 +486,22 @@
 {
 	hipLaunchKernelGGL((k_zq_at<256, KMAX>), dim3(c->cfg.N), dim3(256), 0, c->stream, c->d, base, c->alpha, (const ResolveState *)sp->d_rs, (const unsigned long long *)sp->d_offs);
 }
-static int spec_update_ZQ(isg_ctx *c, SpecCtx *sp, isg_wh base, bool *done)
+static int spec_update_ZQ(isg_ctx *c, SpecCtx *sp, isg_wh base, bool *done, bool pro_done)
 {
 	const int K = c->cfg.K;
 	return spec_update_ZQ_with(c, sp, base, done,
 				   [&](float *alo, float *ahi) { kdispatch(KL_ZQ(), K, [&](auto km) { spec_launch_expect<decltype(km)::value>(c, sp, alo, ahi); }); },
 				   [&](int grid) { kdispatch(KL_ZQ(), K, [&](auto km) { spec_launch_probe<decltype(km)::value>(c, sp, base, grid); }); },
-				   [&]() { kdispatch(KL_ZQ(), K, [&](auto km) { spec_launch_at<decltype(km)::value>(c, sp, base); }); });
-}
+				   [&]() { kdispatch(KL_ZQ(), K, [&](auto km) { spec_launch_at<decltype(km)::value>(c, sp, base); }); }, pro_done);
+}
+static int spec_ZQ_prologue_ahead(isg_ctx *c, SpecCtx *sp)
+{
+	const int K = c->cfg.K;
+	c->d.tape = nullptr;
+	c->d.tape_len = 0;
+	bool ready = false;
+	if (spec_ZQ_prologue(c, sp, [&](float *alo, float *ahi) { kdispatch(KL_ZQ(), K, [&](auto km) { spec_launch_expect<decltype(km)::value>(c, sp, alo, ahi); }); }, false, &ready)) return 1;
+	c->zq_pro_ready = ready;
+	ahead_set(&c->ah, AH_EXPECT);
+	return 0;
+}
diff --git a/instruct_amd/csrc/isg_walk_hip.inc b/instruct_amd/csrc/isg_walk_hip.inc
--- a/instruct_amd/csrc/isg_walk_hip.inc
+++ b/instruct_amd/csrc/isg_walk_hip.inc
@@ -224,6 +224,7 @@
 	DevBuf<float> d_tapef;
 	unsigned long long tape_len = 0;
 	bool usable = false;
+	int test_abort = 0;
 	long sweeps = 0, fallbacks = 0, retried = 0;
 };
 
@@ -319,6 +320,7 @@
 	if (p->G < 1) { delete p; return 0; }
 	p->walk.seg_groups = (int)env_int(getenv("INSTRUCT_WALK_SEG"), 12800, 64, INT_MAX);
 	p->walk.kwin = env_double(getenv("INSTRUCT_WALK_K"), p->walk.kwin, 1.0);
+	p->test_abort = (int)env_int(getenv("INSTRUCT_P_TEST_ABORT"), 0);
 	*out = p;
 	HIPCHK(p->d_gam0.alloc((size_t)p->G + 1));
 	HIPCHK(p->d_gidx.alloc(p->NG));
@@ -333,7 +335,21 @@
 	return 0;
 }
 
-static int pdev_update_P_once(isg_ctx *c, PDevCtx *p, bool *done, bool second, bool *again)
+static void pdev_launch_prep(isg_ctx *c, PDevCtx *p)
+{
+	const unsigned nchunk = (unsigned)((p->NG + 1023) / 1024) + 1u;
+	prof_begin(c);
+	hipLaunchKernelGGL(k_pd_gather, dim3(nchunk), dim3(256), 0, c->stream, (const int *)c->d.cnt, (const int *)p->d_gidx, p->NG, p->d_gcnt, p->d_part);
+	hipLaunchKernelGGL(k_pd_scan, dim3(nchunk), dim3(256), 0, c->stream, (const int *)p->d_gcnt, p->NG, (const unsigned *)p->d_part, p->d_gpos);
+	prof_end(c, "k_pd_prep");
+}
+struct MailP {
+	WkState st;
+	unsigned long long tail[2];
+};
+static_assert(sizeof(MailP) <= MAIL_G - MAIL_P, "update_P's slot of the mailbox");
+
+static int pdev_update_P_once(isg_ctx *c, PDevCtx *p, bool *done, bool second, bool *again, bool prepped)
 {
 	*done = false;
 	*again = false;
@@ -343,13 +359,7 @@
 	if (!ok) { p->usable = false; return 0; }
 	WalkRun &w = p->walk;
 	HIPCHK(hipMemsetAsync(w.d_st, 0, sizeof(WkState), c->stream));
-	prof_begin(c);
-	{
-		const unsigned nchunk = (unsigned)((p->NG + 1023) / 1024) + 1u;
-		hipLaunchKernelGGL(k_pd_gather, dim3(nchunk), dim3(256), 0, c->stream, (const int *)c->d.cnt, (const int *)p->d_gidx, p->NG, p->d_gcnt, p->d_part);
-		hipLaunchKernelGGL(k_pd_scan, dim3(nchunk), dim3(256), 0, c->stream, (const int *)p->d_gcnt, p->NG, (const unsigned *)p->d_part, p->d_gpos);
-	}
-	prof_end(c, "k_pd_prep");
+	if (!prepped) pdev_launch_prep(c, p);
 	prof_begin(c);
 	hipLaunchKernelGGL(k_tapef, dim3((unsigned)((p->tape_len + 2047) / 2048)), dim3(256), 0, c->stream, c->d.tab, c->rng, (unsigned long long)p->tape_len, p->d_tapef);
 	prof_end(c, "k_tapef_P");
@@ -366,13 +376,21 @@
 			   (const unsigned long long *)p->d_gpos, (const unsigned long long *)w.d_T, p->G, w.d_st);
 	prof_end(c, "k_pdirich_at");
 	HIPCHK(hipGetLastError());
-	WkState hs;
-	unsigned long long tail[2] = {0, 0};
-	HIPCHK(hipMemcpyAsync(&hs, w.d_st, sizeof(hs), hipMemcpyDeviceToHost, c->stream));
-	HIPCHK(hipMemcpyAsync(&tail[0], p->d_gpos + p->NG, sizeof(unsigned long long), hipMemcpyDeviceToHost, c->stream));
-	HIPCHK(hipMemcpyAsync(&tail[1], w.d_T + p->G, sizeof(unsigned long long), hipMemcpyDeviceToHost, c->stream));
-	HIPCHK(hipStreamSynchronize(c->stream));
+	MailP *m = mail_slot<MailP>(c, MAIL_P);
+	HIPCHK(hipMemcpyAsync(&m->st, w.d_st, sizeof(m->st), hipMemcpyDeviceToHost, c->stream));
+	HIPCHK(hipMemcpyAsync(&m->tail[0], p->d_gpos + p->NG, sizeof(unsigned long long), hipMemcpyDeviceToHost, c->stream));
+	HIPCHK(hipMemcpyAsync(&m->tail[1], w.d_T + p->G, sizeof(unsigned long long), hipMemcpyDeviceToHost, c->stream));
+	if (look_record(c, AH_LOOK_P)) return 1;
+	if (c->la_on) {
+		if (refresh_freqf(c)) return 1;
+		ahead_set(&c->ah, AH_FREQF);
+	}
+	if (look_wait(c, AH_LOOK_P)) return 1;
+	WkState hs = m->st;
+	const unsigned long long tail[2] = {m->tail[0], m->tail[1]};
 	walk_adapt(w, hs);
+	if (p->test_abort > 0 && --p->test_abort == 0) hs.fail |= 8u;
+	if (hs.fail) ahead_wrote_freq(&c->ah);
 	if (!second && hs.fail == 1u) {
 		*again = true;
 		return 0;
@@ -386,11 +404,11 @@
 	*done = true;
 	return 0;
 }
-static int pdev_update_P(isg_ctx *c, PDevCtx *p, bool *done)
+static int pdev_update_P(isg_ctx *c, PDevCtx *p, bool *done, bool prepped = false)
 {
 	bool again = false;
-	if (pdev_update_P_once(c, p, done, false, &again)) return 1;
+	if (pdev_update_P_once(c, p, done, false, &again, prepped)) return 1;
 	if (!again) return 0;
 	p->retried++;
-	return pdev_update_P_once(c, p, done, true, &again);
-}
+	return pdev_update_P_once(c, p, done, true, &again, false);
+}
```

Result: faster. 359.2 iterations/s (median of 6 runs) (+5.1%).
